# yas-sim/pyopenvino

Measured on AMD Instinct MI355X. Metric: images/sec googlenet-v1 fp32 @batch256, higher is better.
Workload: dtype f32

## Files before the change

pyopenvino_amd/csrc/pvhip_common.h:

```cpp
#pragma once
#include <hip/hip_runtime.h>
#include <cstdarg>
#include <cstdint>
#include <cstdio>

#include "../../include/pvhip.h"

namespace pvhip {

constexpr int kMaxStreams = PVHIP_MAX_STREAMS;

struct State {
    bool        ready  = false;
    int         device = -1;
    hipStream_t stream = nullptr;
    hipStream_t streams[kMaxStreams] = {};
    int         current = 0;
    bool        forked  = false;
    bool        capturing = false;
};
State& state();

struct Settings {
    int generation = 0;
    int  conv_kernel    = 0;
    bool conv_winograd  = true;
    int  conv_winograd4 = 1;
    int  conv_winograd5 = 1;
    bool conv_pointwise = true;
    bool conv_stem      = true;
    bool conv_stem_wino = false;
    int  poolconv_prio  = -1;
    int  fuse_poolconv  = 2;
    bool pool3          = true;
    int  stream_nt      = 1;
    int  stream_wg      = 16;
    int  tile_bm = 0, tile_bn = 0;
    int  wtile_m = 2, wtile_n = 1;
    int  conv_lds_pad_kb = 0;
    bool conv_nopw = false;
    int  f16_bm = 0;
    int  f16_c8_wgs = 0;
    int  f16_c8_prod = 0;
    int  f16_c8_reg = 0;
    int  f16_c8_tpw = 0;
    bool lrnpool_wave = false;
    int  dwconv_cols = 1;
    bool conv_novalid = false;
    bool conv_pw16 = false;
    int  multi_bm = 32;
    int  pw_tn = 0;
    int  pw_stagger_pct = 0;
    int  pool3_kb = 16, pool3_stage = 1, pool3_wg = 0, pool3_g = 0, pool3_s = 0, pool3_band = 0;
    bool pool3_verbose = false;
    int  pool_lds_kb = 16;
    int  wino_kb = 0;
    bool wino_small = true;
    int  wino_waves = 8;
    bool wino_ragged = true;
    bool wino_balance = true;
    int  wino_shared = 1;
    int  wino_shared_prio = 1;
    int  wino_shared_old = 1;
    bool wino_shared_odd = true;
    int  wino_shared_lag = 0;
    int  wino_shared_min_tiles = 2048;
    int  conv_ablate = 0, wino4_ablate = 0, pw_ablate = 0, stem_ablate = 0;
    int  tune[8] = {0, 0, 0, 0, 0, 0, 0, 0};
    bool pool3_tuning() const { return pool3_kb != 16 || pool3_stage != 1 || pool3_wg != 0 || pool3_g != 0; }
};
const Settings& settings();
void            load_settings();

int matmul_impl(const float* a, const float* b, float* c, int m, int n, int k, int trans_a, int trans_b, int round_f16);

int fail(int code, const char* fmt, ...);

constexpr int kWave      = 64;
constexpr int kNumCU     = 256;
constexpr int kBlock     = 256;
constexpr int kMaxBlocks = kNumCU * 8;

inline int grid_for(size_t work_items, int per_block = kBlock) {
    size_t b = (work_items + per_block - 1) / per_block;
    if (b < 1) b = 1;
    if (b > (size_t)kMaxBlocks) b = kMaxBlocks;
    return (int)b;
}

struct FastDiv {
    unsigned mul, shift, d;
};
inline FastDiv make_fastdiv(unsigned d) {
    FastDiv f{0u, 0u, d};
    if (d <= 1) return f;
    unsigned s = 0;
    while ((1ull << s) < d) ++s;
    const unsigned long long k = 31ull + s;
    f.mul   = (unsigned)(((1ull << k) + d - 1) / d);
    f.shift = s - 1;
    return f;
}
__device__ __forceinline__ unsigned fdiv(unsigned n, const FastDiv& f) {
    return f.d <= 1 ? n : (__umulhi(n, f.mul) >> f.shift);
}

__device__ __forceinline__ float max3_nan(float a, float b, float c) {
    return __builtin_elementwise_maximum(__builtin_elementwise_maximum(a, b), c);
}


struct ActBounds {
    float lo, hi;
};
__device__ __forceinline__ ActBounds act_bounds(int act, float lo, float hi) {
    ActBounds b;
    b.lo = act == 1 ? 0.0f : (act == 2 ? lo : -__builtin_inff());
    b.hi = act == 2 ? hi : __builtin_inff();
    return b;
}
__device__ __forceinline__ float act_apply(float v, const ActBounds& b) {
    v = (v < b.lo) ? b.lo : v;
    v = (v > b.hi) ? b.hi : v;
    return v;
}
template <int N>
__device__ __forceinline__ void bias_act_n(float (&v)[N], const float (&b)[N], bool has_bias, int act, const ActBounds& ab) {
    if (has_bias) {
#pragma unroll
        for (int i = 0; i < N; ++i) v[i] = v[i] + b[i];
    }
    if (act == 1) {
#pragma unroll
        for (int i = 0; i < N; ++i) v[i] = __builtin_elementwise_maximum(v[i], 0.0f);
    } else if (act != 0) {
#pragma unroll
        for (int i = 0; i < N; ++i) v[i] = (v[i] < ab.lo) ? ab.lo : v[i];
    }
    if (act == 2) {
#pragma unroll
        for (int i = 0; i < N; ++i) v[i] = (v[i] > ab.hi) ? ab.hi : v[i];
    }
}

__device__ __forceinline__ float lrn_pow_f(float d, float beta, int beta_mode) {
    if (beta_mode == 1) {
        const float s = sqrtf(d);
        return s * sqrtf(s);
    }
    if (beta_mode == 2) return sqrtf(d);
    if (beta_mode == 3) return d;
    return powf(d, beta);
}

__device__ __forceinline__ float lrn_div(float x, float d, float beta, int beta_mode) {
    if (beta_mode == 4) return x * __builtin_amdgcn_exp2f(-0.75f * __builtin_amdgcn_logf(d));
    return x / lrn_pow_f(d, beta, beta_mode);
}

inline int lrn_beta_mode(float beta, float bias) {
    if (beta == 0.75f) return bias >= 1e-20f ? 4 : 1;
    if (beta == 0.5f) return 2;
    if (beta == 1.0f) return 3;
    return 0;
}

constexpr bool kConvStoreNT = false;
constexpr bool kConvStoreSC1 = false;
typedef float pv_f4v __attribute__((ext_vector_type(4)));
typedef float pv_f2v __attribute__((ext_vector_type(2)));
__device__ __forceinline__ void conv_store1(float* p, float v) {
#if defined(__HIP_DEVICE_COMPILE__)
    if (kConvStoreSC1) { asm volatile("global_store_dword %0, %1, off sc1" :: "v"(p), "v"(v) : "memory"); return; }
#endif
    if (kConvStoreNT) __builtin_nontemporal_store(v, p);
    else *p = v;
}
__device__ __forceinline__ void conv_store2(float* p, float a, float b) {
    pv_f2v v; v.x = a; v.y = b;
#if defined(__HIP_DEVICE_COMPILE__)
    if (kConvStoreSC1) { asm volatile("global_store_dwordx2 %0, %1, off sc1" :: "v"(p), "v"(v) : "memory"); return; }
#endif
    if (kConvStoreNT) __builtin_nontemporal_store(v, reinterpret_cast<pv_f2v*>(p));
    else *reinterpret_cast<pv_f2v*>(p) = v;
}
__device__ __forceinline__ void conv_store4(float* p, float a, float b, float c, float d) {
    pv_f4v v; v.x = a; v.y = b; v.z = c; v.w = d;
#if defined(__HIP_DEVICE_COMPILE__)
    if (kConvStoreSC1) { asm volatile("global_store_dwordx4 %0, %1, off sc1" :: "v"(p), "v"(v) : "memory"); return; }
#endif
    if (kConvStoreNT) __builtin_nontemporal_store(v, reinterpret_cast<pv_f4v*>(p));
    else *reinterpret_cast<pv_f4v*>(p) = v;
}
template <class V>
__device__ __forceinline__ void conv_storev(V* p, V v) {
#if defined(__HIP_DEVICE_COMPILE__)
    if (kConvStoreSC1) {
        if constexpr (sizeof(V) == 4) { const float f_ = v[0]; asm volatile("global_store_dword %0, %1, off sc1" :: "v"(p), "v"(f_) : "memory"); }
        else if constexpr (sizeof(V) == 8) asm volatile("global_store_dwordx2 %0, %1, off sc1" :: "v"(p), "v"(v) : "memory");
        else asm volatile("global_store_dwordx4 %0, %1, off sc1" :: "v"(p), "v"(v) : "memory");
        return;
    }
#endif
    if (kConvStoreNT) __builtin_nontemporal_store(v, p);
    else *p = v;
}

typedef __attribute__((address_space(3))) void* lds_void_p;
__device__ __forceinline__ void lds_dma_b32(__amdgpu_buffer_rsrc_t r, float* dst, unsigned voff, unsigned soff) {
#if defined(__HIP_DEVICE_COMPILE__)
    const unsigned lds = (unsigned)(unsigned long)(lds_void_p)dst;
    asm volatile("s_mov_b32 m0, %0\n\ts_nop 0\n\tbuffer_load_dword %1, %2, %3 offen lds"
                 :: "s"(lds), "v"(voff), "s"(r), "s"(soff) : "memory");
#endif
}
__device__ __forceinline__ void lds_dma_b128(__amdgpu_buffer_rsrc_t r, float* dst, unsigned voff, unsigned soff) {
#if defined(__HIP_DEVICE_COMPILE__)
    const unsigned lds = (unsigned)(unsigned long)(lds_void_p)dst;
    asm volatile("s_mov_b32 m0, %0\n\ts_nop 0\n\tbuffer_load_dwordx4 %1, %2, %3 offen lds"
                 :: "s"(lds), "v"(voff), "s"(r), "s"(soff) : "memory");
#endif
}
__device__ __forceinline__ void lds_dma_wait_all() { asm volatile("s_waitcnt vmcnt(0)" ::: "memory"); }

}

#define PVHIP_REQUIRE_INIT()                                                          \
    do {                                                                              \
        if (!pvhip::state().ready)                                                    \
            return pvhip::fail(PVHIP_ENOTINIT, "%s: pvhip_init() not called", __func__); \
    } while (0)

#define PVHIP_HIP(call)                                                               \
    do {                                                                              \
        hipError_t e_ = (call);                                                       \
        if (e_ != hipSuccess)                                                         \
            return pvhip::fail(PVHIP_EHIP, "%s: %s -> %s", __func__, #call,           \
                               hipGetErrorString(e_));                                \
    } while (0)

#define PVHIP_CHECK_ARG(cond)                                                         \
    do {                                                                              \
        if (!(cond))                                                                  \
            return pvhip::fail(PVHIP_EINVAL, "%s: argument check failed: %s",         \
                               __func__, #cond);                                      \
    } while (0)

#define PVHIP_LAUNCH_CHECK()                                                          \
    do {                                                                              \
        hipError_t e_ = hipGetLastError();                                            \
        if (e_ != hipSuccess)                                                         \
            return pvhip::fail(PVHIP_EHIP, "%s: kernel launch -> %s", __func__,       \
                               hipGetErrorString(e_));                                \
    } while (0)
```

pyopenvino_amd/csrc/pvhip_norm.hip:

```cpp
#include "pvhip_common.h"

using namespace pvhip;

namespace {

constexpr bool kStreamNT = true;
template <class T>
__device__ __forceinline__ T ldnt(const T* p) { return kStreamNT ? __builtin_nontemporal_load(p) : *p; }
template <class T>
__device__ __forceinline__ void stnt(T* p, T v) { if (kStreamNT) __builtin_nontemporal_store(v, p); else *p = v; }

__device__ __forceinline__ float wave_sum(float v) {
#pragma unroll
    for (int off = kWave / 2; off > 0; off >>= 1) v += __shfl_xor(v, off, kWave);
    return v;
}

constexpr int kSoftmaxPerThread = 8;

__global__ __launch_bounds__(kBlock) void softmax_rows_kernel(const float* __restrict__ x, float* __restrict__ y,
                                                               int rows, int cols) {
    __shared__ float wave_part[kBlock / kWave];
    const int lane = threadIdx.x & (kWave - 1);
    const int wid  = threadIdx.x / kWave;
    for (int r = blockIdx.x; r < rows; r += gridDim.x) {
        const float* __restrict__ xr = x + (size_t)r * cols;
        float* __restrict__       yr = y + (size_t)r * cols;
        float e[kSoftmaxPerThread];
        float part = 0.0f;
        const bool in_regs = cols <= kBlock * kSoftmaxPerThread;
        if (in_regs) {
#pragma unroll
            for (int j = 0; j < kSoftmaxPerThread; ++j) {
                const int c = threadIdx.x + j * kBlock;
                e[j]        = (c < cols) ? expf(xr[c]) : 0.0f;
                part += e[j];
            }
        } else {
            for (int c = threadIdx.x; c < cols; c += kBlock) part += expf(xr[c]);
        }
        part = wave_sum(part);
        __syncthreads();
        if (lane == 0) wave_part[wid] = part;
        __syncthreads();
        float total = 0.0f;
#pragma unroll
        for (int wv = 0; wv < kBlock / kWave; ++wv) total += wave_part[wv];
        if (in_regs) {
#pragma unroll
            for (int j = 0; j < kSoftmaxPerThread; ++j) {
                const int c = threadIdx.x + j * kBlock;
                if (c < cols) yr[c] = e[j] / total;
            }
        } else {
            for (int c = threadIdx.x; c < cols; c += kBlock) yr[c] = expf(xr[c]) / total;
        }
    }
}

template <int SIZE, int VEC, int BETA_MODE>
__global__ __launch_bounds__(kBlock) void lrn_window_kernel(const float* __restrict__ x, float* __restrict__ y, int n,
                                                             int c, int hw, float alpha, float beta, float bias) {
    constexpr int beta_mode = BETA_MODE;
    constexpr int HALF = SIZE / 2;
    constexpr int T    = 8;
    constexpr int E    = 2 * HALF + T;
    static_assert(2 * HALF <= T, "window halo must fit in one chunk");
    typedef float vec_t __attribute__((ext_vector_type(VEC)));
    const int      cols_per_img = hw / VEC;
    const unsigned total        = (unsigned)n * (unsigned)cols_per_img;
    const unsigned stride       = gridDim.x * blockDim.x;
    const int      n_chunks     = c / T;
    const size_t   cstride      = (size_t)hw / VEC;

#define PV_LRN_OUT(j_, ch_)                                                                    \
    {                                                                                          \
        vec_t s_ = ext[(j_)] * ext[(j_)];                                                      \
        _Pragma("unroll") for (int q = 1; q < SIZE; ++q) s_ = s_ + ext[(j_) + q] * ext[(j_) + q]; \
        vec_t o_;                                                                              \
        _Pragma("unroll") for (int v = 0; v < VEC; ++v) {                                      \
            const float d_ = bias + alpha * s_[v];                                             \
            o_[v]          = lrn_div(ext[(j_) + HALF][v], d_, beta, beta_mode);                \
        }                                                                                      \
        stnt(yv + (size_t)(ch_) * cstride, o_);                                                      \
    }

    for (unsigned t = blockIdx.x * blockDim.x + threadIdx.x; t < total; t += stride) {
        const unsigned img  = t / (unsigned)cols_per_img;
        const unsigned col  = t - img * (unsigned)cols_per_img;
        const size_t   base = (size_t)img * c * hw + (size_t)col * VEC;
        const vec_t* __restrict__ xv = reinterpret_cast<const vec_t*>(x + base);
        vec_t* __restrict__       yv = reinterpret_cast<vec_t*>(y + base);
        vec_t ext[E], nxt[T];
#pragma unroll
        for (int j = 0; j < 2 * HALF; ++j) ext[j] = (vec_t)(0.0f);
#pragma unroll
        for (int j = 0; j < T; ++j) ext[2 * HALF + j] = ldnt(xv + (size_t)j * cstride);
        for (int k = 0; k + 1 < n_chunks; ++k) {
            const vec_t* __restrict__ xn = xv + (size_t)(k + 1) * T * cstride;
#pragma unroll
            for (int j = 0; j < T; ++j) nxt[j] = ldnt(xn + (size_t)j * cstride);
            if (k == 0) {
#pragma unroll
                for (int j = HALF; j < T; ++j) PV_LRN_OUT(j, j - HALF)
            } else {
                const int ch0 = k * T - HALF;
#pragma unroll
                for (int j = 0; j < T; ++j) PV_LRN_OUT(j, ch0 + j)
            }
#pragma unroll
            for (int j = 0; j < 2 * HALF; ++j) ext[j] = ext[T + j];
#pragma unroll
            for (int j = 0; j < T; ++j) ext[2 * HALF + j] = nxt[j];
        }
        {
            const int k = n_chunks - 1, ch0 = k * T - HALF;
            if (k == 0) {
#pragma unroll
                for (int j = HALF; j < T; ++j) PV_LRN_OUT(j, j - HALF)
            } else {
#pragma unroll
                for (int j = 0; j < T; ++j) PV_LRN_OUT(j, ch0 + j)
            }
#pragma unroll
            for (int j = 0; j < 2 * HALF; ++j) ext[j] = ext[T + j];
#pragma unroll
            for (int j = 0; j < T; ++j) ext[2 * HALF + j] = (vec_t)(0.0f);
#pragma unroll
            for (int j = 0; j < HALF; ++j) PV_LRN_OUT(j, c - HALF + j)
        }
    }
#undef PV_LRN_OUT
}

struct LrnPoolArgs {
    const float* x;
    float*       y;
    int   n, c, h, w, oh, ow;
    int   pt, pl, hp, wp;
    int   band_rows, n_bands;
    int   plane_l;
    float alpha, beta, bias;
    int   pool4;
    int   abl;
};

template <int SIZE, int VEC, int BETA_MODE, int ST, int NI>
__global__ __launch_bounds__(kBlock) void lrn_maxpool3x3_kernel(LrnPoolArgs a, FastDiv d_bands, FastDiv d_ow) {
    constexpr int beta_mode = BETA_MODE;
    constexpr int HALF = SIZE / 2;
    constexpr int T    = 8;
    constexpr int E    = 2 * HALF + T;
    static_assert(2 * HALF <= T, "window halo must fit in one chunk");
    typedef float vec_t __attribute__((ext_vector_type(VEC)));
    extern __shared__ __attribute__((aligned(16))) float planes[];
#ifdef PVHIP_DIAG
    const int abl = a.abl;
#else
    constexpr int abl = 0;
#endif

    const int tid = threadIdx.x;
    const int img = (int)fdiv(blockIdx.x, d_bands), band = (int)blockIdx.x - img * a.n_bands;
    const int oy0 = band * a.band_rows, oy1 = min(a.oh, oy0 + a.band_rows);
    const int rows_t = oy1 - oy0;
    const int iy_lo = max(0, oy0 * ST - a.pt), iy_hi = min(a.h, (oy1 - 1) * ST + 3 - a.pt);
    const int band_px = (iy_hi - iy_lo) * a.w;
    const int hw = a.h * a.w, ohw = a.oh * a.ow;
    const bool   active  = tid * VEC < band_px;
    const size_t cstride = (size_t)hw / VEC;
    const vec_t* __restrict__ xv =
        reinterpret_cast<const vec_t*>(a.x + (size_t)img * a.c * hw + (size_t)iy_lo * a.w + (active ? tid * VEC : 0));
    float* const mine = planes + tid * VEC;
    const int    n_chunks = a.c / T;
    const int    out_pp   = a.band_rows * a.ow;

#define PV_LRN_TO_LDS(j_, slot_)                                                               \
    {                                                                                          \
        vec_t s_ = ext[(j_)] * ext[(j_)];                                                      \
        _Pragma("unroll") for (int q = 1; q < SIZE; ++q) s_ = s_ + ext[(j_) + q] * ext[(j_) + q]; \
        vec_t o_;                                                                              \
        _Pragma("unroll") for (int v = 0; v < VEC; ++v) {                                      \
            const float d_ = a.bias + a.alpha * s_[v];                                         \
            o_[v]          = (abl & 1) ? ext[(j_) + HALF][v] : lrn_div(ext[(j_) + HALF][v], d_, a.beta, beta_mode); \
        }                                                                                      \
        if (active) *reinterpret_cast<vec_t*>(mine + (slot_) * a.plane_l) = o_;                \
    }

    unsigned tap[NI][9];
    unsigned outo[NI];
    bool     live[NI], zpad[NI];
#pragma unroll
    for (int i = 0; i < NI; ++i) {
        const unsigned rem = (unsigned)(tid + i * kBlock);
        const unsigned oyl = fdiv(rem, d_ow), ox = rem - oyl * (unsigned)a.ow;
        live[i] = (int)rem < out_pp && (int)oyl < rows_t;
        const int oy = oy0 + (int)oyl;
        const int py0 = oy * ST - a.pt, px0 = (int)ox * ST - a.pl;
        const int c0 = min(max(px0, 0), a.w - 1), c1 = min(max(px0 + 1, 0), a.w - 1), c2 = min(max(px0 + 2, 0), a.w - 1);
#pragma unroll
        for (int k = 0; k < 3; ++k) {
            const int r = (min(max(py0 + k, 0), a.h - 1) - iy_lo) * a.w;
            tap[i][3 * k + 0] = live[i] ? (unsigned)(r + c0) * 4u : 0u;
            tap[i][3 * k + 1] = live[i] ? (unsigned)(r + c1) * 4u : 0u;
            tap[i][3 * k + 2] = live[i] ? (unsigned)(r + c2) * 4u : 0u;
        }
        const bool zc = (px0 < 0) || (min((int)ox * ST + 2, a.wp - 1) - a.pl >= a.w);
        const bool zr = (py0 < 0) || (min(oy * ST + 2, a.hp - 1) - a.pt >= a.h);
        zpad[i] = zc || zr;
        outo[i] = (unsigned)(oy * a.ow) + ox;
    }
    float* const yimg = a.y + (size_t)img * a.c * ohw;
    const char* const planes_b = reinterpret_cast<const char*>(planes);
    const unsigned plane_bytes = (unsigned)a.plane_l * 4u;

    unsigned p4_row[3] = {0u, 0u, 0u}, p4_c8 = 0u, p4_out = 0u, p4_z = 0u;
    bool     p4_live = false;
    const int wv4 = tid >> 6;
    if constexpr (VEC == 4 && ST == 2) {
        if (a.pool4 != 0) {
            const int ql = tid & 63, qpr = a.ow >> 2;
            const int oyl = ql / qpr, oxq = ql - oyl * qpr;
            p4_live = oyl < rows_t;
            const int oy = oy0 + (p4_live ? oyl : 0);
            const int py0 = oy * ST, c0 = 8 * oxq;
#pragma unroll
            for (int k = 0; k < 3; ++k) p4_row[k] = (unsigned)((min(py0 + k, a.h - 1) - iy_lo) * a.w + c0) * 4u;
            p4_c8 = (unsigned)(min(c0 + 8, a.w - 1) - c0) * 4u;
            const bool zr = min(oy * ST + 2, a.hp - 1) >= a.h;
#pragma unroll
            for (int j = 0; j < 4; ++j) p4_z |= ((zr || min((4 * oxq + j) * ST + 2, a.wp - 1) >= a.w) ? 1u : 0u) << j;
            p4_out = (unsigned)(oy * a.ow + 4 * oxq);
        }
    }
    auto pool4 = [&](int n_pl, int ch0) {
        __syncthreads();
        if (p4_live && !(abl & 2)) {
            typedef float f4_t __attribute__((ext_vector_type(4)));
            for (int p = wv4; p < n_pl; p += 4) {
                const char* const pb = reinterpret_cast<const char*>(planes) + (unsigned)p * ((unsigned)a.plane_l * 4u);
                float hm[3][4];
#pragma unroll
                for (int k = 0; k < 3; ++k) {
                    const f4_t lo = *reinterpret_cast<const f4_t*>(pb + p4_row[k]), hi = *reinterpret_cast<const f4_t*>(pb + p4_row[k] + 16);
                    const float c8 = *reinterpret_cast<const float*>(pb + p4_row[k] + p4_c8);
                    hm[k][0] = max3_nan(lo[0], lo[1], lo[2]);
                    hm[k][1] = max3_nan(lo[2], lo[3], hi[0]);
                    hm[k][2] = max3_nan(hi[0], hi[1], hi[2]);
                    hm[k][3] = max3_nan(hi[2], hi[3], c8);
                }
                f4_t m;
#pragma unroll
                for (int j = 0; j < 4; ++j) {
                    const float mj = max3_nan(hm[0][j], hm[1][j], hm[2][j]);
                    m[j] = ((p4_z >> j) & 1u) ? max3_nan(mj, 0.0f, 0.0f) : mj;
                }
                if (!(abl & 4)) *reinterpret_cast<f4_t*>(a.y + (size_t)img * a.c * (a.oh * a.ow) + (size_t)(ch0 + p) * (a.oh * a.ow) + p4_out) = m;
            }
        }
        __syncthreads();
    };
    auto pool = [&](int n_pl, int ch0) {
        if constexpr (VEC == 4 && ST == 2) {
            if (a.pool4 != 0) { pool4(n_pl, ch0); return; }
        }
        __syncthreads();
#pragma unroll
        for (int i = 0; i < NI; ++i) {
            if (!live[i] || (abl & 2)) continue;
            float* yo = yimg + (size_t)ch0 * ohw + outo[i];
            unsigned pb = 0u;
            for (int p = 0; p < n_pl; ++p, pb += plane_bytes, yo += ohw) {
                float h[3];
#pragma unroll
                for (int k = 0; k < 3; ++k) {
                    const float v0 = *reinterpret_cast<const float*>(planes_b + pb + tap[i][3 * k + 0]);
                    const float v1 = *reinterpret_cast<const float*>(planes_b + pb + tap[i][3 * k + 1]);
                    const float v2 = *reinterpret_cast<const float*>(planes_b + pb + tap[i][3 * k + 2]);
                    h[k] = max3_nan(v0, v1, v2);
                }
                float m = max3_nan(h[0], h[1], h[2]);
                if (zpad[i]) m = max3_nan(m, 0.0f, 0.0f);
                if (!(abl & 4)) *yo = m;
            }
        }
        __syncthreads();
    };

    vec_t ext[E], nxt[T];
#pragma unroll
    for (int j = 0; j < 2 * HALF; ++j) ext[j] = (vec_t)(0.0f);
#pragma unroll
    for (int j = 0; j < T; ++j) ext[2 * HALF + j] = ldnt(xv + (size_t)j * cstride);
    for (int k = 0; k + 1 < n_chunks; ++k) {
        const vec_t* __restrict__ xn = xv + (size_t)((abl & 8) ? 0 : (k + 1) * T) * cstride;
#pragma unroll
        for (int j = 0; j < T; ++j) nxt[j] = ldnt(xn + (size_t)j * cstride);
        if (k == 0) {
#pragma unroll
            for (int j = HALF; j < T; ++j) PV_LRN_TO_LDS(j, j - HALF)
            pool(T - HALF, 0);
        } else {
#pragma unroll
            for (int j = 0; j < T; ++j) PV_LRN_TO_LDS(j, j)
            pool(T, k * T - HALF);
        }
#pragma unroll
        for (int j = 0; j < 2 * HALF; ++j) ext[j] = ext[T + j];
#pragma unroll
        for (int j = 0; j < T; ++j) ext[2 * HALF + j] = nxt[j];
    }
    {
        const int k = n_chunks - 1;
        if (k == 0) {
#pragma unroll
            for (int j = HALF; j < T; ++j) PV_LRN_TO_LDS(j, j - HALF)
            pool(T - HALF, 0);
        } else {
#pragma unroll
            for (int j = 0; j < T; ++j) PV_LRN_TO_LDS(j, j)
            pool(T, k * T - HALF);
        }
#pragma unroll
        for (int j = 0; j < 2 * HALF; ++j) ext[j] = ext[T + j];
#pragma unroll
        for (int j = 0; j < T; ++j) ext[2 * HALF + j] = (vec_t)(0.0f);
#pragma unroll
        for (int j = 0; j < HALF; ++j) PV_LRN_TO_LDS(j, j)
        pool(HALF, a.c - HALF);
    }
#undef PV_LRN_TO_LDS
}

template <int SIZE, int VEC, int BETA_MODE, int ST, int NI>
__global__ __launch_bounds__(kBlock) void maxpool3x3_lrn_kernel(LrnPoolArgs a, FastDiv d_bands, FastDiv d_ow) {
    constexpr int beta_mode = BETA_MODE;
    constexpr int HALF = SIZE / 2;
    constexpr int T    = 8;
    typedef float vec_t __attribute__((ext_vector_type(VEC)));
    extern __shared__ __attribute__((aligned(16))) float planes[];

    const int tid = threadIdx.x;
    const int img = (int)fdiv(blockIdx.x, d_bands), band = (int)blockIdx.x - img * a.n_bands;
    const int oy0 = band * a.band_rows, oy1 = min(a.oh, oy0 + a.band_rows);
    const int rows_t = oy1 - oy0;
    const int iy_lo = max(0, oy0 * ST - a.pt), iy_hi = min(a.h, (oy1 - 1) * ST + 3 - a.pt);
    const int band_px = (iy_hi - iy_lo) * a.w;
    const int hw = a.h * a.w, ohw = a.oh * a.ow;
    const bool   active  = tid * VEC < band_px;
    const size_t cstride = (size_t)hw / VEC;
    const vec_t* __restrict__ xv =
        reinterpret_cast<const vec_t*>(a.x + (size_t)img * a.c * hw + (size_t)iy_lo * a.w + (active ? tid * VEC : 0));
    float* const mine = planes + tid * VEC;
    const int    n_chunks = a.c / T;
    const int    out_pp   = a.band_rows * a.ow;

    unsigned tap[NI][9];
    unsigned outo[NI];
    bool     live[NI], zpad[NI];
#pragma unroll
    for (int i = 0; i < NI; ++i) {
        const unsigned rem = (unsigned)(tid + i * kBlock);
        const unsigned oyl = fdiv(rem, d_ow), ox = rem - oyl * (unsigned)a.ow;
        live[i] = (int)rem < out_pp && (int)oyl < rows_t;
        const int oy = oy0 + (int)oyl;
        const int py0 = oy * ST - a.pt, px0 = (int)ox * ST - a.pl;
        const int c0 = min(max(px0, 0), a.w - 1), c1 = min(max(px0 + 1, 0), a.w - 1), c2 = min(max(px0 + 2, 0), a.w - 1);
#pragma unroll
        for (int k = 0; k < 3; ++k) {
            const int r = (min(max(py0 + k, 0), a.h - 1) - iy_lo) * a.w;
            tap[i][3 * k + 0] = live[i] ? (unsigned)(r + c0) * 4u : 0u;
            tap[i][3 * k + 1] = live[i] ? (unsigned)(r + c1) * 4u : 0u;
            tap[i][3 * k + 2] = live[i] ? (unsigned)(r + c2) * 4u : 0u;
        }
        const bool zc = (px0 < 0) || (min((int)ox * ST + 2, a.wp - 1) - a.pl >= a.w);
        const bool zr = (py0 < 0) || (min(oy * ST + 2, a.hp - 1) - a.pt >= a.h);
        zpad[i] = zc || zr;
        outo[i] = (unsigned)(oy * a.ow) + ox;
    }
    float* const yimg = a.y + (size_t)img * a.c * ohw;
    const char* const planes_b = reinterpret_cast<const char*>(planes);
    const unsigned plane_bytes = (unsigned)a.plane_l * 4u;

    float win[NI][SIZE];
#pragma unroll
    for (int i = 0; i < NI; ++i)
#pragma unroll
        for (int q = 0; q < SIZE; ++q) win[i][q] = 0.0f;

#define PV_PUSH_EMIT(i_, v_, ch_)                                                              \
    {                                                                                          \
        _Pragma("unroll") for (int q = 0; q + 1 < SIZE; ++q) win[i_][q] = win[i_][q + 1];      \
        win[i_][SIZE - 1] = (v_);                                                              \
        if ((ch_) >= HALF) {                                                                   \
            float s_ = win[i_][0] * win[i_][0];                                                \
            _Pragma("unroll") for (int q = 1; q < SIZE; ++q) s_ = s_ + win[i_][q] * win[i_][q]; \
            const float d_ = a.bias + a.alpha * s_;                                            \
            yimg[(size_t)((ch_) - HALF) * ohw + outo[i_]] = lrn_div(win[i_][HALF], d_, a.beta, beta_mode);    \
        }                                                                                      \
    }

    vec_t cur[T], nxt[T];
#pragma unroll
    for (int j = 0; j < T; ++j) cur[j] = ldnt(xv + (size_t)j * cstride);
    for (int k = 0; k < n_chunks; ++k) {
        if (k + 1 < n_chunks) {
            const vec_t* __restrict__ xn = xv + (size_t)(k + 1) * T * cstride;
#pragma unroll
            for (int j = 0; j < T; ++j) nxt[j] = ldnt(xn + (size_t)j * cstride);
        }
        if (active) {
#pragma unroll
            for (int j = 0; j < T; ++j) *reinterpret_cast<vec_t*>(mine + j * a.plane_l) = cur[j];
        }
        __syncthreads();
#pragma unroll
        for (int i = 0; i < NI; ++i) {
            if (!live[i]) continue;
            unsigned pb = 0u;
#pragma unroll
            for (int p = 0; p < T; ++p, pb += plane_bytes) {
                float h[3];
#pragma unroll
                for (int q = 0; q < 3; ++q) {
                    const float v0 = *reinterpret_cast<const float*>(planes_b + pb + tap[i][3 * q + 0]);
                    const float v1 = *reinterpret_cast<const float*>(planes_b + pb + tap[i][3 * q + 1]);
                    const float v2 = *reinterpret_cast<const float*>(planes_b + pb + tap[i][3 * q + 2]);
                    h[q] = max3_nan(v0, v1, v2);
                }
                float m = max3_nan(h[0], h[1], h[2]);
                if (zpad[i]) m = max3_nan(m, 0.0f, 0.0f);
                const float pooled = m;
                PV_PUSH_EMIT(i, pooled, k * T + p)
            }
        }
        __syncthreads();
#pragma unroll
        for (int j = 0; j < T; ++j) cur[j] = nxt[j];
    }
#pragma unroll
    for (int i = 0; i < NI; ++i) {
        if (!live[i]) continue;
#pragma unroll
        for (int j = 0; j < HALF; ++j) PV_PUSH_EMIT(i, 0.0f, a.c + j)
    }
#undef PV_PUSH_EMIT
}

typedef float floatx32 __attribute__((ext_vector_type(32)));

struct PoolLrnConvArgs {
    LrnPoolArgs  p;
    const float* cw;
    const float* cbias;
    float*       y;
    int   k_out, act;
    float act_lo, act_hi;
};

template <int BETA_MODE, int ST, int KT>
__global__ __launch_bounds__(kBlock) void maxpool3x3_lrn_conv1x1_kernel(PoolLrnConvArgs ca, FastDiv d_bands, FastDiv d_ow) {
    constexpr int beta_mode = BETA_MODE;
    constexpr int SIZE = 5, HALF = SIZE / 2, T = 8, VEC = 4;
    typedef float vec_t __attribute__((ext_vector_type(VEC)));
    extern __shared__ __attribute__((aligned(16))) float planes[];
    const LrnPoolArgs& a = ca.p;
    float* const wl = planes + T * a.plane_l;

    const int tid = threadIdx.x;
    const int lane = tid & (kWave - 1);
    const int img = (int)fdiv(blockIdx.x, d_bands), band = (int)blockIdx.x - img * a.n_bands;
    const int oy0 = band * a.band_rows, oy1 = min(a.oh, oy0 + a.band_rows);
    const int rows_t = oy1 - oy0;
    const int iy_lo = max(0, oy0 * ST - a.pt), iy_hi = min(a.h, (oy1 - 1) * ST + 3 - a.pt);
    const int band_px = (iy_hi - iy_lo) * a.w;
    const int hw = a.h * a.w, ohw = a.oh * a.ow;
    const bool   active  = tid * VEC < band_px;
    const size_t cstride = (size_t)hw / VEC;
    const vec_t* __restrict__ xv =
        reinterpret_cast<const vec_t*>(a.x + (size_t)img * a.c * hw + (size_t)iy_lo * a.w + (active ? tid * VEC : 0));
    float* const mine = planes + tid * VEC;
    const int    n_chunks = a.c / T;
    const int    out_pp   = a.band_rows * a.ow;

    for (int e = tid; e < a.c * 32 * KT; e += kBlock) {
        const int c = e / (32 * KT), k = e - c * (32 * KT);
        wl[e] = k < ca.k_out ? ca.cw[(size_t)k * a.c + c] : 0.0f;
    }

    unsigned tap[9];
    unsigned outo;
    bool     live, zpad;
    {
        const unsigned rem = (unsigned)tid;
        const unsigned oyl = fdiv(rem, d_ow), ox = rem - oyl * (unsigned)a.ow;
        live = (int)rem < out_pp && (int)oyl < rows_t;
        const int oy = oy0 + (int)oyl;
        const int py0 = oy * ST - a.pt, px0 = (int)ox * ST - a.pl;
        const int c0 = min(max(px0, 0), a.w - 1), c1 = min(max(px0 + 1, 0), a.w - 1), c2 = min(max(px0 + 2, 0), a.w - 1);
#pragma unroll
        for (int k = 0; k < 3; ++k) {
            const int r = (min(max(py0 + k, 0), a.h - 1) - iy_lo) * a.w;
            tap[3 * k + 0] = live ? (unsigned)(r + c0) * 4u : 0u;
            tap[3 * k + 1] = live ? (unsigned)(r + c1) * 4u : 0u;
            tap[3 * k + 2] = live ? (unsigned)(r + c2) * 4u : 0u;
        }
        const bool zc = (px0 < 0) || (min((int)ox * ST + 2, a.wp - 1) - a.pl >= a.w);
        const bool zr = (py0 < 0) || (min(oy * ST + 2, a.hp - 1) - a.pt >= a.h);
        zpad = zc || zr;
        outo = live ? (unsigned)(oy * a.ow) + ox : 0xffffffffu;
    }
    const char* const planes_b = reinterpret_cast<const char*>(planes);
    const unsigned plane_bytes = (unsigned)a.plane_l * 4u;
    const float* const wl_lane = wl + (lane & 31);

    float win[SIZE];
#pragma unroll
    for (int q = 0; q < SIZE; ++q) win[q] = 0.0f;
    floatx32 acc[KT];
#pragma unroll
    for (int kt = 0; kt < KT; ++kt)
#pragma unroll
        for (int r = 0; r < 32; ++r) acc[kt][r] = 0.0f;

#define PV_PUSH_MFMA(v_, ch_)                                                                  \
    {                                                                                          \
        _Pragma("unroll") for (int q = 0; q + 1 < SIZE; ++q) win[q] = win[q + 1];              \
        win[SIZE - 1] = (v_);                                                                  \
        if ((ch_) >= HALF) {                                                                   \
            float s_ = win[0] * win[0];                                                        \
            _Pragma("unroll") for (int q = 1; q < SIZE; ++q) s_ = s_ + win[q] * win[q];        \
            const float d_ = a.bias + a.alpha * s_;                                            \
            const float o_ = live ? lrn_div(win[HALF], d_, a.beta, beta_mode) : 0.0f;          \
            const float* const wc_ = wl_lane + ((ch_) - HALF) * (32 * KT);                     \
            _Pragma("unroll") for (int kt = 0; kt < KT; ++kt)                                  \
                acc[kt] = __builtin_amdgcn_mfma_f32_32x32x1f32(wc_[32 * kt], o_, acc[kt], 0, 0, 0); \
        }                                                                                      \
    }

    vec_t cur[T], nxt[T];
#pragma unroll
    for (int j = 0; j < T; ++j) cur[j] = ldnt(xv + (size_t)j * cstride);
    for (int k = 0; k < n_chunks; ++k) {
        if (k + 1 < n_chunks) {
            const vec_t* __restrict__ xn = xv + (size_t)(k + 1) * T * cstride;
#pragma unroll
            for (int j = 0; j < T; ++j) nxt[j] = ldnt(xn + (size_t)j * cstride);
        }
        if (active) {
#pragma unroll
            for (int j = 0; j < T; ++j) *reinterpret_cast<vec_t*>(mine + j * a.plane_l) = cur[j];
        }
        __syncthreads();
        {
            unsigned pb = 0u;
#pragma unroll
            for (int p = 0; p < T; ++p, pb += plane_bytes) {
                float h[3];
#pragma unroll
                for (int q = 0; q < 3; ++q) {
                    const float v0 = *reinterpret_cast<const float*>(planes_b + pb + tap[3 * q + 0]);
                    const float v1 = *reinterpret_cast<const float*>(planes_b + pb + tap[3 * q + 1]);
                    const float v2 = *reinterpret_cast<const float*>(planes_b + pb + tap[3 * q + 2]);
                    h[q] = max3_nan(v0, v1, v2);
                }
                float m = max3_nan(h[0], h[1], h[2]);
                if (zpad) m = max3_nan(m, 0.0f, 0.0f);
                PV_PUSH_MFMA(m, k * T + p)
            }
        }
        __syncthreads();
#pragma unroll
        for (int j = 0; j < T; ++j) cur[j] = nxt[j];
    }
#pragma unroll
    for (int j = 0; j < HALF; ++j) PV_PUSH_MFMA(0.0f, a.c + j)
#undef PV_PUSH_MFMA

    const int h2 = lane >> 5;
    unsigned outo_b[2];
    outo_b[0] = (unsigned)__shfl((int)outo, lane & 31, kWave);
    outo_b[1] = (unsigned)__shfl((int)outo, 32 + (lane & 31), kWave);
    float* const yimg = ca.y + (size_t)img * ca.k_out * ohw;
    const ActBounds ab = act_bounds(ca.act, ca.act_lo, ca.act_hi);
#pragma unroll
    for (int kt = 0; kt < KT; ++kt) {
        float bv[16];
#pragma unroll
        for (int v = 0; v < 16; ++v) {
            const int kk = 32 * kt + 8 * (v >> 2) + 4 * h2 + (v & 3);
            bv[v] = (ca.cbias != nullptr && kk < ca.k_out) ? ca.cbias[kk] : 0.0f;
        }
#pragma unroll
        for (int b = 0; b < 2; ++b) {
            float vv[16];
#pragma unroll
            for (int v = 0; v < 16; ++v) vv[v] = acc[kt][16 * b + v];
            bias_act_n<16>(vv, bv, ca.cbias != nullptr, ca.act, ab);
            if (outo_b[b] != 0xffffffffu) {
#pragma unroll
                for (int v = 0; v < 16; ++v) {
                    const int kk = 32 * kt + 8 * (v >> 2) + 4 * h2 + (v & 3);
                    if (kk < ca.k_out) yimg[(size_t)kk * ohw + outo_b[b]] = vv[v];
                }
            }
        }
    }
}

struct LrnPoolWaveArgs {
    const float* x;
    float*       y;
    int   n, c, h, w, oh, ow;
    int   R, n_bands, rows_in;
    int   cg, n_groups;
    int   lpr, op;
    long  n_items;
    float alpha, beta, bias;
};

template <int BETA_MODE>
__global__ __launch_bounds__(kBlock) void lrn_maxpool3x3_wave_kernel(LrnPoolWaveArgs a) {
    constexpr int T = 4;
    typedef float vec4 __attribute__((ext_vector_type(4)));
    struct V8 { vec4 lo, hi; };
    extern __shared__ __attribute__((aligned(16))) float wave_planes[];
    const int lane = threadIdx.x & (kWave - 1);
    const int wid  = __builtin_amdgcn_readfirstlane(threadIdx.x / kWave);
    const long item = (long)blockIdx.x * (kBlock / kWave) + wid;
    if (item >= a.n_items) return;
    const int g    = (int)(item % a.n_groups);
    const long ib  = item / a.n_groups;
    const int band = (int)(ib % a.n_bands), img = (int)(ib / a.n_bands);
    const int oy0  = band * a.R;
    const int iy0  = 2 * oy0;
    const int c0   = g * a.cg;
    const int hw = a.h * a.w, ohw = a.oh * a.ow;
    const int plane_l = a.rows_in * a.w;
    float* const lds = wave_planes + (size_t)wid * T * plane_l;

    const int  lrow = lane / a.lpr, lcol = (lane - lrow * a.lpr) * 8;
    const bool lact = lrow < a.rows_in && iy0 + lrow < a.h;
    const float* const xl = a.x + (size_t)img * a.c * hw + (size_t)(lact ? (iy0 + lrow) * a.w + lcol : 0);
    float* const lmine = lds + lrow * a.w + lcol;
    const bool lwrite = lrow < a.rows_in;

    const int  prow = lane / a.op, pj = lane - prow * a.op;
    const int  oy = oy0 + prow, ox = 2 * pj;
    const bool pact = prow < a.R && oy < a.oh && ox < a.ow;
    const bool second = ox + 1 < a.ow;
    unsigned roff[3];
#pragma unroll
    for (int k = 0; k < 3; ++k) {
        const int r = 2 * prow + k;
        roff[k] = (unsigned)(((pact && iy0 + r < a.h) ? r : 2 * (pact ? prow : 0)) * a.w + 4 * (pact ? pj : 0));
    }
    const bool col4 = 4 * pj + 4 < a.w;
    float* const yout = a.y + ((size_t)img * a.c) * ohw + (size_t)(pact ? oy * a.ow + ox : 0);

    auto load8 = [&](int ch) -> V8 {
        V8 v;
        if (lact && ch >= 0 && ch < a.c) {
            const vec4* p = reinterpret_cast<const vec4*>(xl + (size_t)ch * hw);
            v.lo = ldnt(p); v.hi = ldnt(p + 1);
        } else {
            v.lo = (vec4)(0.0f); v.hi = (vec4)(0.0f);
        }
        return v;
    };
    V8 win[5], nxt[T];
#pragma unroll
    for (int q = 0; q < 5; ++q) { win[q].lo = (vec4)(0.0f); win[q].hi = (vec4)(0.0f); }
    const int n_chunks = a.cg / T + 1;
#pragma unroll
    for (int j = 0; j < T; ++j) nxt[j] = load8(c0 - 2 + j);
    for (int i = 0; i < n_chunks; ++i) {
        V8 cur[T];
#pragma unroll
        for (int j = 0; j < T; ++j) cur[j] = nxt[j];
        if (i + 1 < n_chunks) {
#pragma unroll
            for (int j = 0; j < T; ++j) nxt[j] = load8(c0 - 2 + T * (i + 1) + j);
        }
#pragma unroll
        for (int j = 0; j < T; ++j) {
#pragma unroll
            for (int q = 0; q < 4; ++q) win[q] = win[q + 1];
            win[4] = cur[j];
            if (i >= 1) {
                vec4 slo = win[0].lo * win[0].lo, shi = win[0].hi * win[0].hi;
#pragma unroll
                for (int q = 1; q < 5; ++q) { slo = slo + win[q].lo * win[q].lo; shi = shi + win[q].hi * win[q].hi; }
                vec4 olo, ohi;
#pragma unroll
                for (int v = 0; v < 4; ++v) {
                    olo[v] = lrn_div(win[2].lo[v], a.bias + a.alpha * slo[v], a.beta, BETA_MODE);
                    ohi[v] = lrn_div(win[2].hi[v], a.bias + a.alpha * shi[v], a.beta, BETA_MODE);
                }
                if (lwrite) {
                    *reinterpret_cast<vec4*>(lmine + j * plane_l) = olo;
                    *reinterpret_cast<vec4*>(lmine + j * plane_l + 4) = ohi;
                }
            }
        }
        if (i == 0) continue;
        __builtin_amdgcn_wave_barrier();
        const int ch0 = c0 + T * (i - 1);
        if (pact) {
#pragma unroll
            for (int p = 0; p < T; ++p) {
                const float* const pl = lds + p * plane_l;
                float m0[3], m1[3];
#pragma unroll
                for (int k = 0; k < 3; ++k) {
                    const vec4  v  = *reinterpret_cast<const vec4*>(pl + roff[k]);
                    const float v4 = col4 ? pl[roff[k] + 4] : v[3];
                    m0[k] = max3_nan(v[0], v[1], v[2]);
                    m1[k] = max3_nan(v[2], v[3], v4);
                }
                const float r0 = max3_nan(m0[0], m0[1], m0[2]), r1 = max3_nan(m1[0], m1[1], m1[2]);
                float* const yo = yout + (size_t)(ch0 + p) * ohw;
                if (second && (a.ow & 1) == 0) *reinterpret_cast<float2*>(yo) = make_float2(r0, r1);
                else { yo[0] = r0; if (second) yo[1] = r1; }
            }
        }
        __builtin_amdgcn_wave_barrier();
    }
}

bool plan_lrn_pool_wave(int n, int c, int h, int w, int size, float beta, float bias, int oh, int ow, int kh, int kw, int sh, int sw, int pt, int pl,
                        int pb, int pr, LrnPoolWaveArgs& a, int& bm) {
    if (n <= 0 || c < 8 || c % 4 != 0 || h < 3 || w < 8 || w % 8 != 0 || oh <= 0 || ow <= 0) return false;
    if (size != 5 || kh != 3 || kw != 3 || sh != 2 || sw != 2 || pt != 0 || pl != 0 || pb != 0 || pr != 0) return false;
    if (2 * (oh - 1) > h - 1 || 2 * (ow - 1) > w - 1 || 2 * (ow - 1) + 2 > w) return false;
    if ((unsigned long long)n * c * h * w >= (1ull << 31)) return false;
    bm = lrn_beta_mode(beta, bias);
    if (bm != 4 && bm != 1) return false;
    const int lpr = w / 8;
    const int R = (kWave / lpr - 1) / 2;
    const int op = (ow + 1) / 2;
    if (R < 1 || R * op > kWave) return false;
    int cg = 0;
    for (int cand = 64; cand >= 16; cand -= 4)
        if (c % cand == 0) { cg = cand; break; }
    if (cg == 0) return false;
    a.n = n; a.c = c; a.h = h; a.w = w; a.oh = oh; a.ow = ow;
    a.R = R; a.n_bands = (oh + R - 1) / R; a.rows_in = 2 * R + 1;
    a.cg = cg; a.n_groups = c / cg; a.lpr = lpr; a.op = op;
    a.n_items = (long)n * a.n_bands * a.n_groups;
    return (size_t)4 * 4 * a.rows_in * w * sizeof(float) <= 64 * 1024;
}

bool plan_lrn_pool(int n, int c, int h, int w, int size, float beta, float bias, int oh, int ow, int kh, int kw, int sh, int sw,
                   int pt, int pl, int pb, int pr, LrnPoolArgs& a, int& vec, int& bm, size_t& lds) {
    if (n <= 0 || c < 8 || c % 8 != 0 || h <= 0 || w <= 0 || oh <= 0 || ow <= 0) return false;
    if (size != 5 || kh != 3 || kw != 3 || sh != sw || (sh != 1 && sh != 2)) return false;
    if (pt < 0 || pl < 0 || pb < 0 || pr < 0 || pt > 2 || pl > 2) return false;
    if ((oh - 1) * sh > pt + h - 1 || (ow - 1) * sw > pl + w - 1) return false;
    if ((unsigned long long)n * c * h * w >= (1ull << 31)) return false;
    bm = lrn_beta_mode(beta, bias);
    if (bm != 4 && bm != 1) return false;
    vec = (w % 4 == 0) ? 4 : 1;
    int rows = (kBlock * vec / w - 3) / sh + 1;
    if (kBlock * vec / w < 3 && h >= 3) return false;
    if (rows < 1) return false;
    if (rows > oh) rows = oh;
    int bands = (oh + rows - 1) / rows;
    rows  = (oh + bands - 1) / bands;
    bands = (oh + rows - 1) / rows;
    int in_rows = (rows - 1) * sh + 3;
    if (in_rows > h) in_rows = h;
    if (in_rows * w > kBlock * vec) return false;
    a.n = n; a.c = c; a.h = h; a.w = w; a.oh = oh; a.ow = ow; a.pt = pt; a.pl = pl; a.hp = h + pt + pb; a.wp = w + pl + pr;
    a.band_rows = rows; a.n_bands = bands;
    if ((rows * ow + kBlock - 1) / kBlock > 4) return false;
    a.plane_l   = (in_rows * w + 3) & ~3;
    lds         = (size_t)8 * a.plane_l * sizeof(float);
    return lds <= 64 * 1024 && (long long)n * bands < (1ll << 31);
}

__global__ __launch_bounds__(kBlock) void lrn_generic_kernel(const float* __restrict__ x, float* __restrict__ y, int n,
                                                              int c, int hw, int size, float alpha, float beta,
                                                              float bias, int beta_mode) {
    const size_t total  = (size_t)n * c * hw;
    const size_t stride = (size_t)gridDim.x * blockDim.x;
    const int    half   = size / 2;
    for (size_t e = (size_t)blockIdx.x * blockDim.x + threadIdx.x; e < total; e += stride) {
        const size_t p   = e % hw;
        const size_t q   = e / hw;
        const int    ch  = (int)(q % c);
        const size_t img = q / c;
        int lo = ch - half, hi = ch + half + 1;
        if (lo < 0) lo = 0;
        if (hi > c) hi = c;
        float s = 0.0f;
        for (int k = lo; k < hi; ++k) {
            const float v = x[(img * c + k) * hw + p];
            s             = (k == lo) ? v * v : s + v * v;
        }
        const float d = bias + alpha * s;
        y[e]          = lrn_div(x[e], d, beta, beta_mode);
    }
}

template <int SIZE, int BETA_MODE>
void launch_lrn_window_b(const float* x, float* y, int n, int c, int hw, float alpha, float beta, float bias) {
    if (hw % 4 == 0) {
        const size_t cols = (size_t)n * (hw / 4);
        hipLaunchKernelGGL((lrn_window_kernel<SIZE, 4, BETA_MODE>), dim3(grid_for(cols)), dim3(kBlock), 0, state().stream, x, y,
                           n, c, hw, alpha, beta, bias);
    } else {
        const size_t cols = (size_t)n * hw;
        hipLaunchKernelGGL((lrn_window_kernel<SIZE, 1, BETA_MODE>), dim3(grid_for(cols)), dim3(kBlock), 0, state().stream, x, y,
                           n, c, hw, alpha, beta, bias);
    }
}

template <int SIZE>
void launch_lrn_window(const float* x, float* y, int n, int c, int hw, float alpha, float beta, float bias, int bm) {
    switch (bm) {
        case 1: launch_lrn_window_b<SIZE, 1>(x, y, n, c, hw, alpha, beta, bias); break;
        case 2: launch_lrn_window_b<SIZE, 2>(x, y, n, c, hw, alpha, beta, bias); break;
        case 3: launch_lrn_window_b<SIZE, 3>(x, y, n, c, hw, alpha, beta, bias); break;
        case 4: launch_lrn_window_b<SIZE, 4>(x, y, n, c, hw, alpha, beta, bias); break;
        default: launch_lrn_window_b<SIZE, 0>(x, y, n, c, hw, alpha, beta, bias); break;
    }
}

}

extern "C" {

int pvhip_softmax_rows_f32(const float* x, float* y, int rows, int cols) {
    PVHIP_REQUIRE_INIT();
    PVHIP_CHECK_ARG(rows >= 0 && cols >= 0);
    if (rows == 0 || cols == 0) return PVHIP_OK;
    PVHIP_CHECK_ARG(x != nullptr && y != nullptr);
    const int g = rows < kMaxBlocks ? rows : kMaxBlocks;
    hipLaunchKernelGGL(softmax_rows_kernel, dim3(g), dim3(kBlock), 0, state().stream, x, y, rows, cols);
    PVHIP_LAUNCH_CHECK();
    return PVHIP_OK;
}

int pvhip_lrn_f32(const float* x, float* y, int n, int c, int hw, int size, float alpha, float beta, float bias) {
    PVHIP_REQUIRE_INIT();
    PVHIP_CHECK_ARG(n >= 0 && c >= 0 && hw >= 0 && size >= 1);
    if ((size_t)n * c * hw == 0) return PVHIP_OK;
    PVHIP_CHECK_ARG(x != nullptr && y != nullptr);
    if ((unsigned long long)n * c * hw >= (1ull << 31))
        return fail(PVHIP_EUNSUPPORTED, "pvhip_lrn_f32: tensor exceeds 2^31 elements");
    const int bm = lrn_beta_mode(beta, bias);
    switch ((c % 8 == 0 && c >= 8) ? size : 0) {
        case 3: launch_lrn_window<3>(x, y, n, c, hw, alpha, beta, bias, bm); break;
        case 5: launch_lrn_window<5>(x, y, n, c, hw, alpha, beta, bias, bm); break;
        case 7: launch_lrn_window<7>(x, y, n, c, hw, alpha, beta, bias, bm); break;
        default:
            hipLaunchKernelGGL(lrn_generic_kernel, dim3(grid_for((size_t)n * c * hw)), dim3(kBlock), 0, state().stream, x, y,
                               n, c, hw, size, alpha, beta, bias, bm);
    }
    PVHIP_LAUNCH_CHECK();
    return PVHIP_OK;
}

int pvhip_lrn_maxpool_supported(int n, int c, int h, int w, int size, float beta, float bias, int oh, int ow, int kh, int kw,
                                int sh, int sw, int pad_top, int pad_left, int pad_bottom, int pad_right) {
    LrnPoolArgs a{};
    int vec = 0, bm = 0;
    size_t lds = 0;
    return plan_lrn_pool(n, c, h, w, size, beta, bias, oh, ow, kh, kw, sh, sw, pad_top, pad_left, pad_bottom, pad_right, a, vec, bm, lds) ? 1 : 0;
}

int pvhip_lrn_maxpool_f32(const float* x, float* y, int n, int c, int h, int w, int size, float alpha, float beta, float bias,
                          int oh, int ow, int kh, int kw, int sh, int sw, int pad_top, int pad_left, int pad_bottom,
                          int pad_right) {
    PVHIP_REQUIRE_INIT();
    {
        LrnPoolWaveArgs wa{};
        int wbm = 0;
        if (settings().lrnpool_wave && plan_lrn_pool_wave(n, c, h, w, size, beta, bias, oh, ow, kh, kw, sh, sw, pad_top, pad_left, pad_bottom, pad_right, wa, wbm)) {
            PVHIP_CHECK_ARG(x != nullptr && y != nullptr);
            wa.x = x; wa.y = y; wa.alpha = alpha; wa.beta = beta; wa.bias = bias;
            const long blocks = (wa.n_items + kBlock / kWave - 1) / (kBlock / kWave);
            if (blocks <= 0x7fffffffL) {
                const size_t wlds = (size_t)(kBlock / kWave) * 4 * wa.rows_in * w * sizeof(float);
                if (wbm == 4) hipLaunchKernelGGL((lrn_maxpool3x3_wave_kernel<4>), dim3((unsigned)blocks), dim3(kBlock), wlds, state().stream, wa);
                else          hipLaunchKernelGGL((lrn_maxpool3x3_wave_kernel<1>), dim3((unsigned)blocks), dim3(kBlock), wlds, state().stream, wa);
                PVHIP_LAUNCH_CHECK();
                return PVHIP_OK;
            }
        }
    }
    LrnPoolArgs a{};
    int vec = 0, bm = 0;
    size_t lds = 0;
    if (!plan_lrn_pool(n, c, h, w, size, beta, bias, oh, ow, kh, kw, sh, sw, pad_top, pad_left, pad_bottom, pad_right, a, vec, bm, lds))
        return fail(PVHIP_EUNSUPPORTED, "pvhip_lrn_maxpool_f32: shape outside the fused kernel (ask pvhip_lrn_maxpool_supported first)");
    PVHIP_CHECK_ARG(x != nullptr && y != nullptr);
    a.x = x; a.y = y; a.alpha = alpha; a.beta = beta; a.bias = bias;
    a.abl = 0;
#ifdef PVHIP_DIAG
    a.abl = settings().conv_ablate;
#endif
    a.pool4 = (vec == 4 && sh == 2 && pad_top == 0 && pad_left == 0 && ow % 4 == 0 && 2 * ow <= w && (ow / 4) * a.band_rows <= kWave && settings().tune[6] != 1) ? 1 : 0;
    const dim3 grid((unsigned)(n * a.n_bands));
    const FastDiv d_bands = make_fastdiv((unsigned)a.n_bands), d_ow = make_fastdiv((unsigned)ow);
    const int ni = (a.band_rows * ow + kBlock - 1) / kBlock;
#define PV_LP(VEC_, BM_, ST_, NI_) \
    hipLaunchKernelGGL((lrn_maxpool3x3_kernel<5, VEC_, BM_, ST_, NI_>), grid, dim3(kBlock), lds, state().stream, a, d_bands, d_ow)
#define PV_LP_NI(VEC_, BM_, ST_)                                  \
    {                                                             \
        if (ni <= 1) PV_LP(VEC_, BM_, ST_, 1);                    \
        else if (ni <= 2) PV_LP(VEC_, BM_, ST_, 2);               \
        else PV_LP(VEC_, BM_, ST_, 4);                            \
    }
    if (ni > 4) return fail(PVHIP_EUNSUPPORTED, "pvhip_lrn_maxpool_f32: more than four pooled outputs per lane and plane");
    if (vec == 4) {
        if (bm == 4) { if (sh == 1) PV_LP_NI(4, 4, 1) else PV_LP_NI(4, 4, 2) }
        else         { if (sh == 1) PV_LP_NI(4, 1, 1) else PV_LP_NI(4, 1, 2) }
    } else {
        if (bm == 4) { if (sh == 1) PV_LP_NI(1, 4, 1) else PV_LP_NI(1, 4, 2) }
        else         { if (sh == 1) PV_LP_NI(1, 1, 1) else PV_LP_NI(1, 1, 2) }
    }
#undef PV_LP_NI
#undef PV_LP
    PVHIP_LAUNCH_CHECK();
    return PVHIP_OK;
}

int pvhip_maxpool_lrn_supported(int n, int c, int h, int w, int oh, int ow, int kh, int kw, int sh, int sw, int pad_top, int pad_left,
                                int pad_bottom, int pad_right, int size, float beta, float bias) {
    LrnPoolArgs a{};
    int vec = 0, bm = 0;
    size_t lds = 0;
    return plan_lrn_pool(n, c, h, w, size, beta, bias, oh, ow, kh, kw, sh, sw, pad_top, pad_left, pad_bottom, pad_right, a, vec, bm, lds) ? 1 : 0;
}

int pvhip_maxpool_lrn_f32(const float* x, float* y, int n, int c, int h, int w, int oh, int ow, int kh, int kw, int sh, int sw,
                          int pad_top, int pad_left, int pad_bottom, int pad_right, int size, float alpha, float beta, float bias) {
    PVHIP_REQUIRE_INIT();
    LrnPoolArgs a{};
    int vec = 0, bm = 0;
    size_t lds = 0;
    if (!plan_lrn_pool(n, c, h, w, size, beta, bias, oh, ow, kh, kw, sh, sw, pad_top, pad_left, pad_bottom, pad_right, a, vec, bm, lds))
        return fail(PVHIP_EUNSUPPORTED, "pvhip_maxpool_lrn_f32: shape outside the fused kernel (ask pvhip_maxpool_lrn_supported first)");
    PVHIP_CHECK_ARG(x != nullptr && y != nullptr);
    a.x = x; a.y = y; a.alpha = alpha; a.beta = beta; a.bias = bias;
    const dim3 grid((unsigned)(n * a.n_bands));
    const FastDiv d_bands = make_fastdiv((unsigned)a.n_bands), d_ow = make_fastdiv((unsigned)ow);
    const int ni = (a.band_rows * ow + kBlock - 1) / kBlock;
    if (ni > 4) return fail(PVHIP_EUNSUPPORTED, "pvhip_maxpool_lrn_f32: more than four pooled outputs per lane and plane");
#define PV_PL(VEC_, BM_, ST_, NI_) \
    hipLaunchKernelGGL((maxpool3x3_lrn_kernel<5, VEC_, BM_, ST_, NI_>), grid, dim3(kBlock), lds, state().stream, a, d_bands, d_ow)
#define PV_PL_NI(VEC_, BM_, ST_)                                  \
    {                                                             \
        if (ni <= 1) PV_PL(VEC_, BM_, ST_, 1);                    \
        else if (ni <= 2) PV_PL(VEC_, BM_, ST_, 2);               \
        else PV_PL(VEC_, BM_, ST_, 4);                            \
    }
    if (vec == 4) {
        if (bm == 4) { if (sh == 1) PV_PL_NI(4, 4, 1) else PV_PL_NI(4, 4, 2) }
        else         { if (sh == 1) PV_PL_NI(4, 1, 1) else PV_PL_NI(4, 1, 2) }
    } else {
        if (bm == 4) { if (sh == 1) PV_PL_NI(1, 4, 1) else PV_PL_NI(1, 4, 2) }
        else         { if (sh == 1) PV_PL_NI(1, 1, 1) else PV_PL_NI(1, 1, 2) }
    }
#undef PV_PL_NI
#undef PV_PL
    PVHIP_LAUNCH_CHECK();
    return PVHIP_OK;
}

static bool plan_pool_lrn_conv(int n, int c, int h, int w, int oh, int ow, int kh, int kw, int sh, int sw, int pt, int pl, int pb, int pr, int size,
                               float beta, float bias, int k_out, LrnPoolArgs& a, int& bm, size_t& lds) {
    int vec = 0;
    if (!plan_lrn_pool(n, c, h, w, size, beta, bias, oh, ow, kh, kw, sh, sw, pt, pl, pb, pr, a, vec, bm, lds)) return false;
    if (vec != 4 || a.band_rows * ow > kBlock || k_out <= 0 || k_out > 64 || c > 64) return false;
    if ((unsigned long long)n * k_out * oh * ow >= (1ull << 31)) return false;
    lds += (size_t)c * 32 * ((k_out + 31) / 32) * sizeof(float);
    return lds <= 64 * 1024;
}

int pvhip_maxpool_lrn_conv1x1_supported(int n, int c, int h, int w, int oh, int ow, int kh, int kw, int sh, int sw, int pad_top, int pad_left,
                                        int pad_bottom, int pad_right, int size, float beta, float bias, int k_out) {
    LrnPoolArgs a{};
    int bm = 0;
    size_t lds = 0;
    return plan_pool_lrn_conv(n, c, h, w, oh, ow, kh, kw, sh, sw, pad_top, pad_left, pad_bottom, pad_right, size, beta, bias, k_out, a, bm, lds) ? 1 : 0;
}

int pvhip_maxpool_lrn_conv1x1_f32(const float* x, const float* w_oihw, float* y, int n, int c, int h, int w, int oh, int ow, int kh, int kw, int sh, int sw,
                                  int pad_top, int pad_left, int pad_bottom, int pad_right, int size, float alpha, float beta, float bias,
                                  int k_out, const float* conv_bias, int act, float act_lo, float act_hi) {
    PVHIP_REQUIRE_INIT();
    PoolLrnConvArgs ca{};
    int bm = 0;
    size_t lds = 0;
    if (!plan_pool_lrn_conv(n, c, h, w, oh, ow, kh, kw, sh, sw, pad_top, pad_left, pad_bottom, pad_right, size, beta, bias, k_out, ca.p, bm, lds))
        return fail(PVHIP_EUNSUPPORTED, "pvhip_maxpool_lrn_conv1x1_f32: shape outside the fused kernel (ask pvhip_maxpool_lrn_conv1x1_supported first)");
    PVHIP_CHECK_ARG(x != nullptr && w_oihw != nullptr && y != nullptr && act >= 0 && act <= 2);
    ca.p.x = x; ca.p.y = nullptr; ca.p.alpha = alpha; ca.p.beta = beta; ca.p.bias = bias;
    ca.cw = w_oihw; ca.cbias = conv_bias; ca.y = y; ca.k_out = k_out; ca.act = act; ca.act_lo = act_lo; ca.act_hi = act_hi;
    const dim3 grid((unsigned)(n * ca.p.n_bands));
    const FastDiv d_bands = make_fastdiv((unsigned)ca.p.n_bands), d_ow = make_fastdiv((unsigned)ow);
    const int kt = (k_out + 31) / 32;
#define PV_PLC(BM_, ST_, KT_) hipLaunchKernelGGL((maxpool3x3_lrn_conv1x1_kernel<BM_, ST_, KT_>), grid, dim3(kBlock), lds, state().stream, ca, d_bands, d_ow)
    if (bm == 4) {
        if (sh == 1) { if (kt == 1) PV_PLC(4, 1, 1); else PV_PLC(4, 1, 2); }
        else         { if (kt == 1) PV_PLC(4, 2, 1); else PV_PLC(4, 2, 2); }
    } else {
        if (sh == 1) { if (kt == 1) PV_PLC(1, 1, 1); else PV_PLC(1, 1, 2); }
        else         { if (kt == 1) PV_PLC(1, 2, 1); else PV_PLC(1, 2, 2); }
    }
#undef PV_PLC
    PVHIP_LAUNCH_CHECK();
    return PVHIP_OK;
}


}
```

pyopenvino_amd/csrc/pvhip_runtime.hip:

```cpp
#include <cstdlib>
#include <cstring>
#include <map>
#include <mutex>
#include <unordered_map>
#include <vector>

#include "pvhip_common.h"

namespace pvhip {

State& state() {
    static State s;
    return s;
}

static Settings g_settings;
const Settings& settings() {
    if (g_settings.generation == 0) load_settings();
    return g_settings;
}

void load_settings() {
    Settings s;
    s.generation = g_settings.generation + 1;
    auto env   = [](const char* name) -> const char* { const char* e = getenv(name); return (e != nullptr && e[0] != 0) ? e : nullptr; };
    auto is0   = [&](const char* name) { const char* e = env(name); return e != nullptr && e[0] == '0'; };
    auto num   = [&](const char* name, int dflt) { const char* e = env(name); return e != nullptr ? atoi(e) : dflt; };
    auto tri   = [&](const char* name) { const char* e = env(name); return e == nullptr ? 1 : (e[0] == '0' ? 0 : (e[0] == 'f' ? 2 : 1)); };
    s.conv_winograd  = !is0("PVHIP_CONV_WINOGRAD");
    s.conv_winograd4 = tri("PVHIP_CONV_WINOGRAD4");
    s.conv_winograd5 = tri("PVHIP_CONV_WINOGRAD5");
    s.conv_pointwise = !is0("PVHIP_CONV_POINTWISE");
    s.conv_stem      = !is0("PVHIP_CONV_STEM");
    { const char* e = env("PVHIP_CONV_STEM_WINO"); s.conv_stem_wino = e != nullptr && e[0] == '1'; }
    for (int i = 0; i < 8; ++i) {
        char name[16];
        snprintf(name, sizeof(name), "PVHIP_TUNE%d", i);
        s.tune[i] = num(name, 0);
    }
    if (const char* e = env("PVHIP_FUSE_POOLCONV")) s.fuse_poolconv = e[0] == '0' ? 0 : (e[0] == '4' ? 4 : (e[0] == '1' ? 1 : 2));
    s.pool3 = !(env("PVHIP_POOL3") != nullptr && num("PVHIP_POOL3", 1) == 0);
    s.stream_nt = num("PVHIP_STREAM_NT", 1);
    s.stream_wg = num("PVHIP_STREAM_WG", 16);
    if (s.stream_wg < 1) s.stream_wg = 1;
    if (s.stream_wg > 64) s.stream_wg = 64;
    s.conv_lds_pad_kb = num("PVHIP_CONV_LDS_PAD_KB", 0);
    s.conv_nopw = env("PVHIP_CONV_NOPW") != nullptr;
    s.conv_novalid = env("PVHIP_CONV_NOVALID") != nullptr;
    s.dwconv_cols = (int)num("PVHIP_DWCONV_COLS", 1);
    { const int b = num("PVHIP_CONV_F16_BM", 0); s.f16_bm = (b == 32 || b == 64 || b == 128) ? b : 0; }
    s.f16_c8_wgs = num("PVHIP_CONV_F16_C8_WGS", 0);
    s.f16_c8_prod = num("PVHIP_CONV_F16_C8_PROD", 0);
    s.f16_c8_reg = num("PVHIP_CONV_F16_C8_REG", 0);
    s.f16_c8_tpw = num("PVHIP_CONV_F16_C8_TPW", 0);
    s.lrnpool_wave = num("PVHIP_LRNPOOL_WAVE", 0) != 0;
    { const int v = num("PVHIP_CONV_MULTI_BM", 32); s.multi_bm = (v == 64 || v == 128) ? v : 32; }
    s.pw_stagger_pct = num("PVHIP_PW_STAGGER", 0);
    s.pw_tn = num("PVHIP_PW_TN", 0);
    s.pool3_kb    = num("PVHIP_POOL3_KB", 16);
    s.pool3_stage = num("PVHIP_POOL3_STAGE", 1) != 0;
    s.pool3_wg    = num("PVHIP_POOL3_WG", 0);
    if (const char* e = env("PVHIP_POOL3_CFG")) {
        int g = 0, sg = 0, band = 0;
        if (sscanf(e, "%d,%d,%d", &g, &sg, &band) == 3 && g > 0 && sg > 0 && band > 0) { s.pool3_g = g; s.pool3_s = sg; s.pool3_band = band; }
    }
    s.pool3_verbose = env("PVHIP_POOL3_VERBOSE") != nullptr;
    s.pool_lds_kb   = num("PVHIP_POOL_LDS_KB", 16);
    { const int v = num("PVHIP_WINO_KB", 0); s.wino_kb = (v == 32 || v == 64) ? v : 0; }
    s.wino_small = !is0("PVHIP_WINO_SMALL");
    s.wino_waves = num("PVHIP_WINO_WAVES", 8) == 4 ? 4 : 8;
    s.wino_balance = num("PVHIP_WINO_BALANCE", 1) != 0;
    s.wino_ragged = num("PVHIP_WINO_RAGGED", 1) != 0;
    s.wino_shared = num("PVHIP_WINO_SHARED", 1);
    s.wino_shared_min_tiles = num("PVHIP_WINO_SHARED_MIN_TILES", 2048);
    s.wino_shared_lag = num("PVHIP_WINO_SHARED_LAG", 0);
    s.wino_shared_prio = num("PVHIP_WINO_SHARED_PRIO", 1);
    s.wino_shared_odd = num("PVHIP_WINO_SHARED_ODD", 1) != 0;
    s.poolconv_prio = num("PVHIP_POOLCONV_PRIO", -1);
    s.wino_shared_old = num("PVHIP_WINO_SHARED_OLD", 1);
#ifdef PVHIP_DIAG
    if (const char* e = env("PVHIP_CONV_KERNEL")) s.conv_kernel = strcmp(e, "lds") == 0 ? 1 : (strcmp(e, "wave") == 0 ? 2 : 0);
    if (const char* e = env("PVHIP_CONV_TILE")) {
        int bm = 0, bn = 0;
        if (sscanf(e, "%dx%d", &bm, &bn) == 2 && (bm == 32 || bm == 64 || bm == 128) && (bn == 128 || bn == 256)) { s.tile_bm = bm; s.tile_bn = bn; }
    }
    if (const char* e = env("PVHIP_CONV_WTILE")) sscanf(e, "%dx%d", &s.wtile_m, &s.wtile_n);
    s.conv_pw16 = env("PVHIP_CONV_PW") != nullptr;
    s.conv_ablate  = num("PVHIP_CONV_ABLATE", 0);
    s.wino4_ablate = num("PVHIP_WINO4_ABLATE", 0);
    s.pw_ablate    = num("PVHIP_PW_ABLATE", 0);
    s.stem_ablate  = num("PVHIP_STEM_ABLATE", 0);
#endif
    g_settings = s;
}

static thread_local char g_err[512] = "no error";

int fail(int code, const char* fmt, ...) {
    va_list ap;
    va_start(ap, fmt);
    vsnprintf(g_err, sizeof(g_err), fmt, ap);
    va_end(ap);
    return code;
}

namespace {
struct Pool {
    std::mutex                                  mu;
    struct Live { size_t bytes; int epoch; bool captured; };
    std::unordered_map<void*, Live>             live;
    std::map<size_t, std::vector<void*>>        cached;
    std::vector<std::pair<void*, size_t>>       deferred;
    int                                                     next_epoch = 1, current_epoch = 0;
    std::unordered_map<int, std::vector<std::pair<void*, size_t>>> parked;
    size_t                                      bytes_live = 0, bytes_cached = 0;
    std::vector<std::pair<void*, size_t>>       capture_keep;
};
Pool& pool() {
    static Pool p;
    return p;
}
inline size_t round_up(size_t b) {
    const size_t q = 512;
    return b == 0 ? q : (b + q - 1) / q * q;
}

int sync_all_streams() {
    State& s = state();
    for (int i = 0; i < kMaxStreams; ++i)
        if (s.streams[i] != nullptr) {
            hipError_t e = hipStreamSynchronize(s.streams[i]);
            if (e != hipSuccess) return fail(PVHIP_EHIP, "hipStreamSynchronize(stream %d) -> %s", i, hipGetErrorString(e));
        }
    Pool& p = pool();
    std::lock_guard<std::mutex> g(p.mu);
    for (auto& blk : p.deferred) {
        p.cached[blk.second].push_back(blk.first);
        p.bytes_cached += blk.second;
    }
    p.deferred.clear();
    s.forked = s.current != 0;
    return PVHIP_OK;
}

struct HostBlocks {
    std::mutex               mu;
    std::map<uintptr_t, size_t> live;
};
HostBlocks& host_blocks() {
    static HostBlocks h;
    return h;
}
}
}

using namespace pvhip;

extern "C" {

int pvhip_abi_version(void) { return PVHIP_ABI_VERSION; }

const char* pvhip_last_error(void) { return g_err; }

int pvhip_device_count(int* count) {
    PVHIP_CHECK_ARG(count != nullptr);
    int n = 0;
    hipError_t e = hipGetDeviceCount(&n);
    if (e != hipSuccess) {
        *count = 0;
        return fail(PVHIP_EHIP, "hipGetDeviceCount -> %s", hipGetErrorString(e));
    }
    *count = n;
    return PVHIP_OK;
}

int pvhip_init(int device) {
    State& s = state();
    if (s.ready) {
        if (s.device == device) return PVHIP_OK;
        return fail(PVHIP_EINVAL, "pvhip_init: already initialised on device %d", s.device);
    }
    int n = 0;
    PVHIP_HIP(hipGetDeviceCount(&n));
    if (device < 0 || device >= n)
        return fail(PVHIP_EINVAL, "pvhip_init: device %d out of range (%d visible)", device, n);
    PVHIP_HIP(hipSetDevice(device));
    PVHIP_HIP(hipStreamCreateWithFlags(&s.streams[0], hipStreamNonBlocking));
    s.stream  = s.streams[0];
    s.current = 0;
    s.forked  = false;
    s.device = device;
    s.ready  = true;
    load_settings();
    return PVHIP_OK;
}

int pvhip_settings_reload(void) {
    load_settings();
    return PVHIP_OK;
}

int pvhip_pool_release(void) {
    PVHIP_REQUIRE_INIT();
    if (int rc = sync_all_streams()) return rc;
    Pool& p = pool();
    std::lock_guard<std::mutex> g(p.mu);
    for (auto& kv : p.cached)
        for (void* ptr : kv.second) (void)hipFree(ptr);
    p.cached.clear();
    p.bytes_cached = 0;
    return PVHIP_OK;
}

int pvhip_shutdown(void) {
    State& s = state();
    if (!s.ready) return PVHIP_OK;
    (void)pvhip_comm_destroy();
    (void)pvhip_pool_release();
    {
        HostBlocks& h = host_blocks();
        std::lock_guard<std::mutex> g(h.mu);
        for (auto& kv : h.live) (void)hipHostFree((void*)kv.first);
        h.live.clear();
    }
    {
        Pool& p = pool();
        std::lock_guard<std::mutex> g(p.mu);
        for (auto& kv : p.live) (void)hipFree(kv.first);
        p.live.clear();
        for (auto& kv : p.parked)
            for (auto& blk : kv.second) (void)hipFree(blk.first);
        p.parked.clear();
        for (auto& blk : p.deferred) (void)hipFree(blk.first);
        p.deferred.clear();
        p.current_epoch = 0;
        p.bytes_live = 0;
    }
    for (int i = 0; i < kMaxStreams; ++i)
        if (s.streams[i] != nullptr) {
            (void)hipStreamDestroy(s.streams[i]);
            s.streams[i] = nullptr;
        }
    s.stream  = nullptr;
    s.current = 0;
    s.forked  = false;
    s.ready  = false;
    s.device = -1;
    return PVHIP_OK;
}

int pvhip_device_name(char* buf, size_t buflen) {
    PVHIP_REQUIRE_INIT();
    PVHIP_CHECK_ARG(buf != nullptr && buflen > 0);
    hipDeviceProp_t prop;
    PVHIP_HIP(hipGetDeviceProperties(&prop, state().device));
    const char* name = prop.name[0] != 0 ? prop.name : (strncmp(prop.gcnArchName, "gfx950", 6) == 0 ? "AMD Instinct MI355X-class (gfx950)" : "AMD GPU");
    snprintf(buf, buflen, "%s (%s, %d CUs)", name, prop.gcnArchName, prop.multiProcessorCount);
    return PVHIP_OK;
}

int pvhip_malloc(void** ptr, size_t bytes) {
    PVHIP_REQUIRE_INIT();
    PVHIP_CHECK_ARG(ptr != nullptr);
    const size_t rb = round_up(bytes);
    Pool&        p  = pool();
    std::lock_guard<std::mutex> g(p.mu);
    auto it = p.cached.find(rb);
    if (it != p.cached.end() && !it->second.empty()) {
        *ptr = it->second.back();
        it->second.pop_back();
        p.bytes_cached -= rb;
    } else {
        if (state().capturing)
            return fail(PVHIP_EHIP, "pvhip_malloc(%zu bytes): the pool has no such block while a pass is being captured into a graph "
                                    "(run the pass eagerly first: steady-state inference allocates nothing new)", rb);
        void*      d = nullptr;
        hipError_t e = hipMalloc(&d, rb);
        if (e != hipSuccess) {
            (void)hipGetLastError();
            for (int i = 0; i < kMaxStreams; ++i)
                if (state().streams[i] != nullptr) (void)hipStreamSynchronize(state().streams[i]);
            for (auto& blk : p.deferred) {
                p.cached[blk.second].push_back(blk.first);
                p.bytes_cached += blk.second;
            }
            p.deferred.clear();
            for (auto& kv : p.cached)
                for (void* c : kv.second) (void)hipFree(c);
            p.cached.clear();
            p.bytes_cached = 0;
            e = hipMalloc(&d, rb);
            if (e != hipSuccess)
                return fail(PVHIP_EHIP, "pvhip_malloc(%zu bytes) -> %s", rb, hipGetErrorString(e));
        }
        *ptr = d;
    }
    p.live[*ptr] = Pool::Live{rb, p.current_epoch, state().capturing};
    p.bytes_live += rb;
    return PVHIP_OK;
}

int pvhip_free(void* ptr) {
    if (ptr == nullptr) return PVHIP_OK;
    if (!state().ready) return PVHIP_OK;
    Pool& p = pool();
    std::lock_guard<std::mutex> g(p.mu);
    auto it = p.live.find(ptr);
    if (it == p.live.end()) return fail(PVHIP_EINVAL, "pvhip_free: %p is not a live pvhip block", ptr);
    const size_t rb    = it->second.bytes;
    const int    epoch = it->second.epoch;
    const bool   captured = it->second.captured;
    p.live.erase(it);
    p.bytes_live -= rb;
    if (state().capturing && captured) {
        p.capture_keep.emplace_back(ptr, rb);
        return PVHIP_OK;
    }
    if (epoch != 0) {
        auto open = p.parked.find(epoch);
        if (open != p.parked.end()) {
            open->second.emplace_back(ptr, rb);
            return PVHIP_OK;
        }
    } else if (state().forked) {
        p.deferred.emplace_back(ptr, rb);
        return PVHIP_OK;
    }
    p.cached[rb].push_back(ptr);
    p.bytes_cached += rb;
    return PVHIP_OK;
}

int pvhip_pool_epoch_begin(int* epoch) {
    PVHIP_REQUIRE_INIT();
    PVHIP_CHECK_ARG(epoch != nullptr);
    Pool& p = pool();
    std::lock_guard<std::mutex> g(p.mu);
    *epoch          = p.next_epoch++;
    p.current_epoch = *epoch;
    p.parked[*epoch];
    return PVHIP_OK;
}

int pvhip_pool_epoch_dispatched(void) {
    PVHIP_REQUIRE_INIT();
    Pool& p = pool();
    std::lock_guard<std::mutex> g(p.mu);
    p.current_epoch = 0;
    return PVHIP_OK;
}

int pvhip_pool_epoch_end(int epoch) {
    PVHIP_REQUIRE_INIT();
    Pool& p = pool();
    std::lock_guard<std::mutex> g(p.mu);
    auto it = p.parked.find(epoch);
    if (it == p.parked.end()) return fail(PVHIP_EINVAL, "pvhip_pool_epoch_end: epoch %d is not open", epoch);
    for (auto& blk : it->second) {
        p.cached[blk.second].push_back(blk.first);
        p.bytes_cached += blk.second;
    }
    p.parked.erase(it);
    if (p.current_epoch == epoch) p.current_epoch = 0;
    return PVHIP_OK;
}

int pvhip_pool_stats(size_t* bytes_in_use, size_t* bytes_cached) {
    Pool& p = pool();
    std::lock_guard<std::mutex> g(p.mu);
    if (bytes_in_use) *bytes_in_use = p.bytes_live;
    if (bytes_cached) *bytes_cached = p.bytes_cached;
    return PVHIP_OK;
}

int pvhip_memcpy_h2d(void* dst, const void* src, size_t bytes) {
    PVHIP_REQUIRE_INIT();
    if (bytes == 0) return PVHIP_OK;
    PVHIP_CHECK_ARG(dst != nullptr && src != nullptr);
    PVHIP_HIP(hipMemcpyAsync(dst, src, bytes, hipMemcpyHostToDevice, state().stream));
    PVHIP_HIP(hipStreamSynchronize(state().stream));
    return PVHIP_OK;
}

int pvhip_memcpy_d2h(void* dst, const void* src, size_t bytes) {
    PVHIP_REQUIRE_INIT();
    if (bytes == 0) return PVHIP_OK;
    PVHIP_CHECK_ARG(dst != nullptr && src != nullptr);
    PVHIP_HIP(hipMemcpyAsync(dst, src, bytes, hipMemcpyDeviceToHost, state().stream));
    PVHIP_HIP(hipStreamSynchronize(state().stream));
    if (state().forked && state().current == 0) return sync_all_streams();
    return PVHIP_OK;
}

void* pvhip_host_alloc(size_t bytes) {
    if (!state().ready || bytes == 0) return nullptr;
    void* p = nullptr;
    if (hipHostMalloc(&p, bytes, hipHostMallocDefault) != hipSuccess) { (void)hipGetLastError(); return nullptr; }
    HostBlocks& h = host_blocks();
    std::lock_guard<std::mutex> g(h.mu);
    h.live[(uintptr_t)p] = bytes;
    return p;
}

int pvhip_host_free(void* p) {
    PVHIP_REQUIRE_INIT();
    if (p == nullptr) return PVHIP_OK;
    {
        HostBlocks& h = host_blocks();
        std::lock_guard<std::mutex> g(h.mu);
        if (h.live.erase((uintptr_t)p) == 0) return fail(PVHIP_EINVAL, "pvhip_host_free: %p is not a live pvhip_host_alloc block", p);
    }
    PVHIP_HIP(hipHostFree(p));
    return PVHIP_OK;
}

int pvhip_host_stats(size_t* blocks, size_t* bytes) {
    HostBlocks& h = host_blocks();
    std::lock_guard<std::mutex> g(h.mu);
    size_t total = 0;
    for (auto& kv : h.live) total += kv.second;
    if (blocks) *blocks = h.live.size();
    if (bytes) *bytes = total;
    return PVHIP_OK;
}

int pvhip_memcpy_h2d_async(void* dst, const void* src, size_t bytes) {
    PVHIP_REQUIRE_INIT();
    if (bytes == 0) return PVHIP_OK;
    PVHIP_CHECK_ARG(dst != nullptr && src != nullptr);
    if (state().capturing) return fail(PVHIP_EINVAL, "pvhip_memcpy_h2d_async: a pass is being captured into a graph (uploads stay outside it)");
    {
        HostBlocks& h = host_blocks();
        std::lock_guard<std::mutex> g(h.mu);
        const uintptr_t a = (uintptr_t)src;
        auto it = h.live.upper_bound(a);
        const bool inside = it != h.live.begin() && (--it, a + bytes <= it->first + it->second);
        if (!inside)
            return fail(PVHIP_EINVAL, "pvhip_memcpy_h2d_async: source %p (+%zu bytes) is not page-locked memory from pvhip_host_alloc", src, bytes);
    }
    PVHIP_HIP(hipMemcpyAsync(dst, src, bytes, hipMemcpyHostToDevice, state().stream));
    return PVHIP_OK;
}

int pvhip_memcpy_d2d(void* dst, const void* src, size_t bytes) {
    PVHIP_REQUIRE_INIT();
    if (bytes == 0) return PVHIP_OK;
    PVHIP_CHECK_ARG(dst != nullptr && src != nullptr);
    PVHIP_HIP(hipMemcpyAsync(dst, src, bytes, hipMemcpyDeviceToDevice, state().stream));
    return PVHIP_OK;
}

int pvhip_memset(void* dst, int byte, size_t bytes) {
    PVHIP_REQUIRE_INIT();
    if (bytes == 0) return PVHIP_OK;
    PVHIP_CHECK_ARG(dst != nullptr);
    PVHIP_HIP(hipMemsetAsync(dst, byte, bytes, state().stream));
    return PVHIP_OK;
}

int pvhip_sync(void) {
    PVHIP_REQUIRE_INIT();
    if (state().capturing) return fail(PVHIP_EINVAL, "pvhip_sync: a pass is being captured into a graph (nothing executes until it is replayed)");
    return sync_all_streams();
}

int pvhip_stream_select(int index) {
    PVHIP_REQUIRE_INIT();
    State& s = state();
    if (index < 0 || index >= kMaxStreams)
        return fail(PVHIP_EINVAL, "pvhip_stream_select: stream %d outside 0..%d", index, kMaxStreams - 1);
    if (s.streams[index] == nullptr) PVHIP_HIP(hipStreamCreateWithFlags(&s.streams[index], hipStreamNonBlocking));
    s.stream  = s.streams[index];
    s.current = index;
    if (index != 0) s.forked = true;
    return PVHIP_OK;
}

int pvhip_stream_wait_event(void* ev) {
    PVHIP_REQUIRE_INIT();
    PVHIP_CHECK_ARG(ev != nullptr);
    PVHIP_HIP(hipStreamWaitEvent(state().stream, (hipEvent_t)ev, 0));
    return PVHIP_OK;
}

int pvhip_event_create_untimed(void** ev) {
    PVHIP_REQUIRE_INIT();
    PVHIP_CHECK_ARG(ev != nullptr);
    hipEvent_t e;
    PVHIP_HIP(hipEventCreateWithFlags(&e, hipEventDisableTiming));
    *ev = (void*)e;
    return PVHIP_OK;
}

int pvhip_event_create(void** ev) {
    PVHIP_REQUIRE_INIT();
    PVHIP_CHECK_ARG(ev != nullptr);
    hipEvent_t e;
    PVHIP_HIP(hipEventCreate(&e));
    *ev = (void*)e;
    return PVHIP_OK;
}

int pvhip_event_destroy(void* ev) {
    if (ev == nullptr || !state().ready) return PVHIP_OK;
    PVHIP_HIP(hipEventDestroy((hipEvent_t)ev));
    return PVHIP_OK;
}

int pvhip_event_record(void* ev) {
    PVHIP_REQUIRE_INIT();
    PVHIP_CHECK_ARG(ev != nullptr);
    PVHIP_HIP(hipEventRecord((hipEvent_t)ev, state().stream));
    return PVHIP_OK;
}

int pvhip_event_sync(void* ev) {
    PVHIP_REQUIRE_INIT();
    PVHIP_CHECK_ARG(ev != nullptr);
    PVHIP_HIP(hipEventSynchronize((hipEvent_t)ev));
    return PVHIP_OK;
}

int pvhip_event_elapsed_ms(void* start, void* stop, float* ms) {
    PVHIP_REQUIRE_INIT();
    PVHIP_CHECK_ARG(start != nullptr && stop != nullptr && ms != nullptr);
    PVHIP_HIP(hipEventElapsedTime(ms, (hipEvent_t)start, (hipEvent_t)stop));
    return PVHIP_OK;
}

struct GraphExec {
    hipGraphExec_t                        exec = nullptr;
    std::vector<std::pair<void*, size_t>> keep;
};

int pvhip_graph_begin_capture(void) {
    PVHIP_REQUIRE_INIT();
    if (state().capturing) return fail(PVHIP_EINVAL, "pvhip_graph_begin_capture: a capture is already open");
    PVHIP_HIP(hipStreamBeginCapture(state().stream, hipStreamCaptureModeRelaxed));
    state().capturing = true;
    return PVHIP_OK;
}

int pvhip_graph_capture_status(int* status) {
    PVHIP_REQUIRE_INIT();
    PVHIP_CHECK_ARG(status != nullptr);
    hipStreamCaptureStatus st = hipStreamCaptureStatusNone;
    PVHIP_HIP(hipStreamIsCapturing(state().stream, &st));
    *status = st == hipStreamCaptureStatusActive ? 1 : (st == hipStreamCaptureStatusInvalidated ? 2 : 0);
    return PVHIP_OK;
}

int pvhip_graph_end_capture(void** graph_exec) {
    PVHIP_REQUIRE_INIT();
    PVHIP_CHECK_ARG(graph_exec != nullptr);
    if (!state().capturing) return fail(PVHIP_EINVAL, "pvhip_graph_end_capture: no capture is open");
    state().capturing = false;
    GraphExec* ge = new GraphExec;
    {
        Pool& p = pool();
        std::lock_guard<std::mutex> g(p.mu);
        ge->keep.swap(p.capture_keep);
    }
    auto release = [&]() {
        Pool& p = pool();
        std::lock_guard<std::mutex> g(p.mu);
        for (auto& blk : ge->keep) { p.cached[blk.second].push_back(blk.first); p.bytes_cached += blk.second; }
        delete ge;
    };
    hipGraph_t g = nullptr;
    hipStreamCaptureStatus cst = hipStreamCaptureStatusNone;
    const hipError_t qe = hipStreamIsCapturing(state().stream, &cst);
    if (getenv("PVHIP_GRAPH_VERBOSE") != nullptr) fprintf(stderr, "pvhip_graph_end_capture: hipStreamIsCapturing -> %d, status %d\n", (int)qe, (int)cst);
    hipError_t e = hipStreamEndCapture(state().stream, &g);
    if (getenv("PVHIP_GRAPH_VERBOSE") != nullptr) fprintf(stderr, "pvhip_graph_end_capture: hipStreamEndCapture -> %d, graph %p\n", (int)e, (void*)g);
    if (e == hipSuccess && (g == nullptr || cst != hipStreamCaptureStatusActive)) e = hipErrorStreamCaptureInvalidated;
    if (e != hipSuccess) {
        if (g != nullptr) (void)hipGraphDestroy(g);
        release();
        (void)hipGetLastError();
        return fail(PVHIP_EHIP, "hipStreamEndCapture -> %s (capture status %d)", hipGetErrorString(e), (int)cst);
    }
    if (getenv("PVHIP_GRAPH_VERBOSE") != nullptr) {
        size_t n_nodes = 0;
        (void)hipGraphGetNodes(g, nullptr, &n_nodes);
        fprintf(stderr, "pvhip_graph_end_capture: %zu nodes\n", n_nodes);
    }
    e = hipGraphInstantiate(&ge->exec, g, nullptr, nullptr, 0);
    (void)hipGraphDestroy(g);
    if (e != hipSuccess) { release(); return fail(PVHIP_EHIP, "hipGraphInstantiate -> %s", hipGetErrorString(e)); }
    *graph_exec = (void*)ge;
    return PVHIP_OK;
}

int pvhip_graph_launch(void* graph_exec) {
    PVHIP_REQUIRE_INIT();
    PVHIP_CHECK_ARG(graph_exec != nullptr);
    PVHIP_HIP(hipGraphLaunch(static_cast<GraphExec*>(graph_exec)->exec, state().stream));
    return PVHIP_OK;
}

int pvhip_graph_destroy(void* graph_exec) {
    if (graph_exec == nullptr) return PVHIP_OK;
    GraphExec* ge = static_cast<GraphExec*>(graph_exec);
    if (state().ready) {
        (void)sync_all_streams();
        if (ge->exec != nullptr) (void)hipGraphExecDestroy(ge->exec);
        Pool& p = pool();
        std::lock_guard<std::mutex> g(p.mu);
        for (auto& blk : ge->keep) { p.cached[blk.second].push_back(blk.first); p.bytes_cached += blk.second; }
    }
    delete ge;
    return PVHIP_OK;
}

}
```

Before: 56020.

## Make LRN+maxpool kernels persistent band walkers with halo-row carry and prefetch

Turns the fused LRN+maxpool and maxpool+LRN+conv1x1 kernels into persistent workgroups, each walking a contiguous range of (image, band) items. The first channel chunk of the next band is prefetched while the current band finishes. When consecutive bands share a boundary input row, that row's LRN output is kept in extra LDS and reused, so the overlapping halo row is neither reloaded nor recomputed. The grid is sized from LDS capacity per CU, and the kernels raise their dynamic LDS limit. This adds LDS pressure, code complexity and a risk of load imbalance.

New measurement: 55080. 0.983x the previous value.

```diff
diff --git a/pyopenvino_amd/csrc/pvhip_common.h b/pyopenvino_amd/csrc/pvhip_common.h
--- a/pyopenvino_amd/csrc/pvhip_common.h
+++ b/pyopenvino_amd/csrc/pvhip_common.h
@@ -45,6 +45,7 @@
     int  f16_c8_reg = 0;
     int  f16_c8_tpw = 0;
     bool lrnpool_wave = false;
+    int  band_wgs = 0;
     int  dwconv_cols = 1;
     bool conv_novalid = false;
     bool conv_pw16 = false;
diff --git a/pyopenvino_amd/csrc/pvhip_norm.hip b/pyopenvino_amd/csrc/pvhip_norm.hip
--- a/pyopenvino_amd/csrc/pvhip_norm.hip
+++ b/pyopenvino_amd/csrc/pvhip_norm.hip
@@ -143,7 +143,34 @@
     float alpha, beta, bias;
     int   pool4;
     int   abl;
+    int   items;
+    int   carry_l;
 };
+
+struct BandGeom {
+    int img, band, oy0, oy1, iy_lo, iy_hi;
+};
+template <int ST>
+__device__ __forceinline__ BandGeom band_geom(const LrnPoolArgs& a, int item, const FastDiv& d_bands) {
+    BandGeom g;
+    g.img   = (int)fdiv((unsigned)item, d_bands);
+    g.band  = item - g.img * a.n_bands;
+    g.oy0   = g.band * a.band_rows;
+    g.oy1   = min(a.oh, g.oy0 + a.band_rows);
+    g.iy_lo = max(0, g.oy0 * ST - a.pt);
+    g.iy_hi = min(a.h, (g.oy1 - 1) * ST + 3 - a.pt);
+    return g;
+}
+template <int ST>
+__device__ __forceinline__ bool band_carried(const LrnPoolArgs& a, const BandGeom& p, const BandGeom& g) {
+    return a.carry_l != 0 && g.img == p.img && g.band == p.band + 1 && g.iy_lo == p.iy_hi - 1 && g.iy_hi - g.iy_lo >= 2 && g.oy0 * ST - a.pt >= 0;
+}
+__device__ __forceinline__ void band_range(int items, int& item, int& item_end) {
+    const int g_ = (int)gridDim.x, b_ = (int)blockIdx.x;
+    const int per = items / g_, extra = items - per * g_;
+    item     = b_ * per + min(b_, extra);
+    item_end = item + per + (b_ < extra ? 1 : 0);
+}
 
 template <int SIZE, int VEC, int BETA_MODE, int ST, int NI>
 __global__ __launch_bounds__(kBlock) void lrn_maxpool3x3_kernel(LrnPoolArgs a, FastDiv d_bands, FastDiv d_ow) {
@@ -153,12 +180,224 @@
     constexpr int E    = 2 * HALF + T;
     static_assert(2 * HALF <= T, "window halo must fit in one chunk");
     typedef float vec_t __attribute__((ext_vector_type(VEC)));
+    typedef float f4_t __attribute__((ext_vector_type(4)));
     extern __shared__ __attribute__((aligned(16))) float planes[];
 #ifdef PVHIP_DIAG
     const int abl = a.abl;
 #else
     constexpr int abl = 0;
 #endif
+
+    const int tid = threadIdx.x;
+    int item, item_end;
+    band_range(a.items, item, item_end);
+    if (item >= item_end) return;
+    const int hw = a.h * a.w, ohw = a.oh * a.ow;
+    const size_t cstride = (size_t)hw / VEC;
+    float* const mine = planes + tid * VEC;
+    float* const carry = planes + T * a.plane_l;
+    const int    n_chunks = a.c / T;
+    const int    out_pp   = a.band_rows * a.ow;
+    const char* const planes_b = reinterpret_cast<const char*>(planes);
+    const unsigned plane_bytes = (unsigned)a.plane_l * 4u;
+    const unsigned carry_b     = (unsigned)(T * a.plane_l) * 4u;
+    const int wv4 = tid >> 6;
+
+    auto src = [&](const BandGeom& g, bool carried, bool& active) -> const vec_t* {
+        active = tid * VEC < (g.iy_hi - g.iy_lo) * a.w && !(carried && tid * VEC < a.w);
+        return reinterpret_cast<const vec_t*>(a.x + (size_t)g.img * a.c * hw + (size_t)g.iy_lo * a.w + (active ? tid * VEC : (carried ? a.w : 0)));
+    };
+
+#define PV_LRN_TO_LDS(j_, slot_)                                                               \
+    {                                                                                          \
+        vec_t s_ = ext[(j_)] * ext[(j_)];                                                      \
+        _Pragma("unroll") for (int q = 1; q < SIZE; ++q) s_ = s_ + ext[(j_) + q] * ext[(j_) + q]; \
+        vec_t o_;                                                                              \
+        _Pragma("unroll") for (int v = 0; v < VEC; ++v) {                                      \
+            const float d_ = a.bias + a.alpha * s_[v];                                         \
+            o_[v]          = (abl & 1) ? ext[(j_) + HALF][v] : lrn_div(ext[(j_) + HALF][v], d_, a.beta, beta_mode); \
+        }                                                                                      \
+        if (active) *reinterpret_cast<vec_t*>(mine + (slot_) * a.plane_l) = o_;                \
+    }
+
+    BandGeom g = band_geom<ST>(a, item, d_bands);
+    bool carried = false, active;
+    const vec_t* __restrict__ xv = src(g, false, active);
+    vec_t ext[E], nxt[T];
+#pragma unroll
+    for (int j = 0; j < T; ++j) nxt[j] = ldnt(xv + (size_t)j * cstride);
+
+    for (;;) {
+        const bool     has_next = item + 1 < item_end;
+        const BandGeom gn = has_next ? band_geom<ST>(a, item + 1, d_bands) : g;
+        const bool     carry_out = has_next && band_carried<ST>(a, g, gn);
+        bool           active_n = false;
+        const vec_t* __restrict__ xvn = has_next ? src(gn, carry_out, active_n) : xv;
+
+        const int oy0 = g.oy0, iy_lo = g.iy_lo, img = g.img;
+        const int rows_t = g.oy1 - g.oy0;
+        const int last0 = (g.iy_hi - g.iy_lo - 1) * a.w;
+
+        unsigned tap[NI][9];
+        unsigned outo[NI];
+        bool     live[NI], zpad[NI];
+#pragma unroll
+        for (int i = 0; i < NI; ++i) {
+            const unsigned rem = (unsigned)(tid + i * kBlock);
+            const unsigned oyl = fdiv(rem, d_ow), ox = rem - oyl * (unsigned)a.ow;
+            live[i] = (int)rem < out_pp && (int)oyl < rows_t;
+            const int oy = oy0 + (int)oyl;
+            const int py0 = oy * ST - a.pt, px0 = (int)ox * ST - a.pl;
+            const int c0 = min(max(px0, 0), a.w - 1), c1 = min(max(px0 + 1, 0), a.w - 1), c2 = min(max(px0 + 2, 0), a.w - 1);
+#pragma unroll
+            for (int k = 0; k < 3; ++k) {
+                const int r = (min(max(py0 + k, 0), a.h - 1) - iy_lo) * a.w;
+                tap[i][3 * k + 0] = live[i] ? (unsigned)(r + c0) * 4u : 0u;
+                tap[i][3 * k + 1] = live[i] ? (unsigned)(r + c1) * 4u : 0u;
+                tap[i][3 * k + 2] = live[i] ? (unsigned)(r + c2) * 4u : 0u;
+            }
+            const bool zc = (px0 < 0) || (min((int)ox * ST + 2, a.wp - 1) - a.pl >= a.w);
+            const bool zr = (py0 < 0) || (min(oy * ST + 2, a.hp - 1) - a.pt >= a.h);
+            zpad[i] = zc || zr;
+            outo[i] = (unsigned)(oy * a.ow) + ox;
+        }
+        float* const yimg = a.y + (size_t)img * a.c * ohw;
+
+        unsigned p4_row[3] = {0u, 0u, 0u}, p4_c8 = 0u, p4_out = 0u, p4_z = 0u, p4_s0 = plane_bytes, p4_ch = 0u;
+        bool     p4_live = false;
+        if constexpr (VEC == 4 && ST == 2) {
+            if (a.pool4 != 0) {
+                const int ql = tid & 63, qpr = a.ow >> 2;
+                const int oyl = ql / qpr, oxq = ql - oyl * qpr;
+                p4_live = oyl < rows_t;
+                const int oy = oy0 + (p4_live ? oyl : 0);
+                const int py0 = oy * ST, c0 = 8 * oxq;
+#pragma unroll
+                for (int k = 0; k < 3; ++k) p4_row[k] = (unsigned)((min(py0 + k, a.h - 1) - iy_lo) * a.w + c0) * 4u;
+                if (carried && p4_live && oyl == 0) { p4_row[0] = carry_b + (unsigned)c0 * 4u; p4_s0 = p4_ch = (unsigned)a.w * 4u; }
+                p4_c8 = (unsigned)(min(c0 + 8, a.w - 1) - c0) * 4u;
+                const bool zr = min(oy * ST + 2, a.hp - 1) >= a.h;
+#pragma unroll
+                for (int j = 0; j < 4; ++j) p4_z |= ((zr || min((4 * oxq + j) * ST + 2, a.wp - 1) >= a.w) ? 1u : 0u) << j;
+                p4_out = (unsigned)(oy * a.ow + 4 * oxq);
+            }
+        }
+        auto pool4 = [&](int n_pl, int ch0) {
+            __syncthreads();
+            for (int p = wv4; p < n_pl; p += 4) {
+                const char* const pb = planes_b + (unsigned)p * plane_bytes;
+                if (p4_live && !(abl & 2)) {
+                    float hm[3][4];
+#pragma unroll
+                    for (int k = 0; k < 3; ++k) {
+                        const char* const rb = k == 0 ? planes_b + p4_row[0] + (unsigned)p * p4_s0 + (unsigned)ch0 * p4_ch : pb + p4_row[k];
+                        const f4_t lo = *reinterpret_cast<const f4_t*>(rb), hi = *reinterpret_cast<const f4_t*>(rb + 16);
+                        const float c8 = *reinterpret_cast<const float*>(rb + p4_c8);
+                        hm[k][0] = max3_nan(lo[0], lo[1], lo[2]);
+                        hm[k][1] = max3_nan(lo[2], lo[3], hi[0]);
+                        hm[k][2] = max3_nan(hi[0], hi[1], hi[2]);
+                        hm[k][3] = max3_nan(hi[2], hi[3], c8);
+                    }
+                    f4_t m;
+#pragma unroll
+                    for (int j = 0; j < 4; ++j) {
+                        const float mj = max3_nan(hm[0][j], hm[1][j], hm[2][j]);
+                        m[j] = ((p4_z >> j) & 1u) ? max3_nan(mj, 0.0f, 0.0f) : mj;
+                    }
+                    if (!(abl & 4)) *reinterpret_cast<f4_t*>(a.y + (size_t)img * a.c * (a.oh * a.ow) + (size_t)(ch0 + p) * (a.oh * a.ow) + p4_out) = m;
+                }
+                if (carry_out) {
+                    for (int q = tid & 63; q < (a.w >> 2); q += kWave)
+                        *reinterpret_cast<f4_t*>(carry + (ch0 + p) * a.carry_l + 4 * q) = *reinterpret_cast<const f4_t*>(planes + p * a.plane_l + last0 + 4 * q);
+                }
+            }
+            __syncthreads();
+        };
+        auto pool = [&](int n_pl, int ch0) {
+            if constexpr (VEC == 4 && ST == 2) {
+                if (a.pool4 != 0) { pool4(n_pl, ch0); return; }
+            }
+            __syncthreads();
+#pragma unroll
+            for (int i = 0; i < NI; ++i) {
+                if (!live[i] || (abl & 2)) continue;
+                float* yo = yimg + (size_t)ch0 * ohw + outo[i];
+                unsigned pb = 0u;
+                for (int p = 0; p < n_pl; ++p, pb += plane_bytes, yo += ohw) {
+                    float h[3];
+#pragma unroll
+                    for (int k = 0; k < 3; ++k) {
+                        const float v0 = *reinterpret_cast<const float*>(planes_b + pb + tap[i][3 * k + 0]);
+                        const float v1 = *reinterpret_cast<const float*>(planes_b + pb + tap[i][3 * k + 1]);
+                        const float v2 = *reinterpret_cast<const float*>(planes_b + pb + tap[i][3 * k + 2]);
+                        h[k] = max3_nan(v0, v1, v2);
+                    }
+                    float m = max3_nan(h[0], h[1], h[2]);
+                    if (zpad[i]) m = max3_nan(m, 0.0f, 0.0f);
+                    if (!(abl & 4)) *yo = m;
+                }
+            }
+            __syncthreads();
+        };
+
+#pragma unroll
+        for (int j = 0; j < 2 * HALF; ++j) ext[j] = (vec_t)(0.0f);
+#pragma unroll
+        for (int j = 0; j < T; ++j) ext[2 * HALF + j] = nxt[j];
+        for (int k = 0; k + 1 < n_chunks; ++k) {
+            const vec_t* __restrict__ xn = xv + (size_t)((abl & 8) ? 0 : (k + 1) * T) * cstride;
+#pragma unroll
+            for (int j = 0; j < T; ++j) nxt[j] = ldnt(xn + (size_t)j * cstride);
+            if (k == 0) {
+#pragma unroll
+                for (int j = HALF; j < T; ++j) PV_LRN_TO_LDS(j, j - HALF)
+                pool(T - HALF, 0);
+            } else {
+#pragma unroll
+                for (int j = 0; j < T; ++j) PV_LRN_TO_LDS(j, j)
+                pool(T, k * T - HALF);
+            }
+#pragma unroll
+            for (int j = 0; j < 2 * HALF; ++j) ext[j] = ext[T + j];
+#pragma unroll
+            for (int j = 0; j < T; ++j) ext[2 * HALF + j] = nxt[j];
+        }
+        {
+            if (has_next) {
+#pragma unroll
+                for (int j = 0; j < T; ++j) nxt[j] = ldnt(xvn + (size_t)j * cstride);
+            }
+            const int k = n_chunks - 1;
+            if (k == 0) {
+#pragma unroll
+                for (int j = HALF; j < T; ++j) PV_LRN_TO_LDS(j, j - HALF)
+                pool(T - HALF, 0);
+            } else {
+#pragma unroll
+                for (int j = 0; j < T; ++j) PV_LRN_TO_LDS(j, j)
+                pool(T, k * T - HALF);
+            }
+#pragma unroll
+            for (int j = 0; j < 2 * HALF; ++j) ext[j] = ext[T + j];
+#pragma unroll
+            for (int j = 0; j < T; ++j) ext[2 * HALF + j] = (vec_t)(0.0f);
+#pragma unroll
+            for (int j = 0; j < HALF; ++j) PV_LRN_TO_LDS(j, j)
+            pool(HALF, a.c - HALF);
+        }
+        if (!has_next) break;
+        ++item; g = gn; carried = carry_out; active = active_n; xv = xvn;
+    }
+#undef PV_LRN_TO_LDS
+}
+
+template <int SIZE, int VEC, int BETA_MODE, int ST, int NI>
+__global__ __launch_bounds__(kBlock) void maxpool3x3_lrn_kernel(LrnPoolArgs a, FastDiv d_bands, FastDiv d_ow) {
+    constexpr int beta_mode = BETA_MODE;
+    constexpr int HALF = SIZE / 2;
+    constexpr int T    = 8;
+    typedef float vec_t __attribute__((ext_vector_type(VEC)));
+    extern __shared__ __attribute__((aligned(16))) float planes[];
 
     const int tid = threadIdx.x;
     const int img = (int)fdiv(blockIdx.x, d_bands), band = (int)blockIdx.x - img * a.n_bands;
@@ -175,186 +414,6 @@
     const int    n_chunks = a.c / T;
     const int    out_pp   = a.band_rows * a.ow;
 
-#define PV_LRN_TO_LDS(j_, slot_)                                                               \
-    {                                                                                          \
-        vec_t s_ = ext[(j_)] * ext[(j_)];                                                      \
-        _Pragma("unroll") for (int q = 1; q < SIZE; ++q) s_ = s_ + ext[(j_) + q] * ext[(j_) + q]; \
-        vec_t o_;                                                                              \
-        _Pragma("unroll") for (int v = 0; v < VEC; ++v) {                                      \
-            const float d_ = a.bias + a.alpha * s_[v];                                         \
-            o_[v]          = (abl & 1) ? ext[(j_) + HALF][v] : lrn_div(ext[(j_) + HALF][v], d_, a.beta, beta_mode); \
-        }                                                                                      \
-        if (active) *reinterpret_cast<vec_t*>(mine + (slot_) * a.plane_l) = o_;                \
-    }
-
-    unsigned tap[NI][9];
-    unsigned outo[NI];
-    bool     live[NI], zpad[NI];
-#pragma unroll
-    for (int i = 0; i < NI; ++i) {
-        const unsigned rem = (unsigned)(tid + i * kBlock);
-        const unsigned oyl = fdiv(rem, d_ow), ox = rem - oyl * (unsigned)a.ow;
-        live[i] = (int)rem < out_pp && (int)oyl < rows_t;
-        const int oy = oy0 + (int)oyl;
-        const int py0 = oy * ST - a.pt, px0 = (int)ox * ST - a.pl;
-        const int c0 = min(max(px0, 0), a.w - 1), c1 = min(max(px0 + 1, 0), a.w - 1), c2 = min(max(px0 + 2, 0), a.w - 1);
-#pragma unroll
-        for (int k = 0; k < 3; ++k) {
-            const int r = (min(max(py0 + k, 0), a.h - 1) - iy_lo) * a.w;
-            tap[i][3 * k + 0] = live[i] ? (unsigned)(r + c0) * 4u : 0u;
-            tap[i][3 * k + 1] = live[i] ? (unsigned)(r + c1) * 4u : 0u;
-            tap[i][3 * k + 2] = live[i] ? (unsigned)(r + c2) * 4u : 0u;
-        }
-        const bool zc = (px0 < 0) || (min((int)ox * ST + 2, a.wp - 1) - a.pl >= a.w);
-        const bool zr = (py0 < 0) || (min(oy * ST + 2, a.hp - 1) - a.pt >= a.h);
-        zpad[i] = zc || zr;
-        outo[i] = (unsigned)(oy * a.ow) + ox;
-    }
-    float* const yimg = a.y + (size_t)img * a.c * ohw;
-    const char* const planes_b = reinterpret_cast<const char*>(planes);
-    const unsigned plane_bytes = (unsigned)a.plane_l * 4u;
-
-    unsigned p4_row[3] = {0u, 0u, 0u}, p4_c8 = 0u, p4_out = 0u, p4_z = 0u;
-    bool     p4_live = false;
-    const int wv4 = tid >> 6;
-    if constexpr (VEC == 4 && ST == 2) {
-        if (a.pool4 != 0) {
-            const int ql = tid & 63, qpr = a.ow >> 2;
-            const int oyl = ql / qpr, oxq = ql - oyl * qpr;
-            p4_live = oyl < rows_t;
-            const int oy = oy0 + (p4_live ? oyl : 0);
-            const int py0 = oy * ST, c0 = 8 * oxq;
-#pragma unroll
-            for (int k = 0; k < 3; ++k) p4_row[k] = (unsigned)((min(py0 + k, a.h - 1) - iy_lo) * a.w + c0) * 4u;
-            p4_c8 = (unsigned)(min(c0 + 8, a.w - 1) - c0) * 4u;
-            const bool zr = min(oy * ST + 2, a.hp - 1) >= a.h;
-#pragma unroll
-            for (int j = 0; j < 4; ++j) p4_z |= ((zr || min((4 * oxq + j) * ST + 2, a.wp - 1) >= a.w) ? 1u : 0u) << j;
-            p4_out = (unsigned)(oy * a.ow + 4 * oxq);
-        }
-    }
-    auto pool4 = [&](int n_pl, int ch0) {
-        __syncthreads();
-        if (p4_live && !(abl & 2)) {
-            typedef float f4_t __attribute__((ext_vector_type(4)));
-            for (int p = wv4; p < n_pl; p += 4) {
-                const char* const pb = reinterpret_cast<const char*>(planes) + (unsigned)p * ((unsigned)a.plane_l * 4u);
-                float hm[3][4];
-#pragma unroll
-                for (int k = 0; k < 3; ++k) {
-                    const f4_t lo = *reinterpret_cast<const f4_t*>(pb + p4_row[k]), hi = *reinterpret_cast<const f4_t*>(pb + p4_row[k] + 16);
-                    const float c8 = *reinterpret_cast<const float*>(pb + p4_row[k] + p4_c8);
-                    hm[k][0] = max3_nan(lo[0], lo[1], lo[2]);
-                    hm[k][1] = max3_nan(lo[2], lo[3], hi[0]);
-                    hm[k][2] = max3_nan(hi[0], hi[1], hi[2]);
-                    hm[k][3] = max3_nan(hi[2], hi[3], c8);
-                }
-                f4_t m;
-#pragma unroll
-                for (int j = 0; j < 4; ++j) {
-                    const float mj = max3_nan(hm[0][j], hm[1][j], hm[2][j]);
-                    m[j] = ((p4_z >> j) & 1u) ? max3_nan(mj, 0.0f, 0.0f) : mj;
-                }
-                if (!(abl & 4)) *reinterpret_cast<f4_t*>(a.y + (size_t)img * a.c * (a.oh * a.ow) + (size_t)(ch0 + p) * (a.oh * a.ow) + p4_out) = m;
-            }
-        }
-        __syncthreads();
-    };
-    auto pool = [&](int n_pl, int ch0) {
-        if constexpr (VEC == 4 && ST == 2) {
-            if (a.pool4 != 0) { pool4(n_pl, ch0); return; }
-        }
-        __syncthreads();
-#pragma unroll
-        for (int i = 0; i < NI; ++i) {
-            if (!live[i] || (abl & 2)) continue;
-            float* yo = yimg + (size_t)ch0 * ohw + outo[i];
-            unsigned pb = 0u;
-            for (int p = 0; p < n_pl; ++p, pb += plane_bytes, yo += ohw) {
-                float h[3];
-#pragma unroll
-                for (int k = 0; k < 3; ++k) {
-                    const float v0 = *reinterpret_cast<const float*>(planes_b + pb + tap[i][3 * k + 0]);
-                    const float v1 = *reinterpret_cast<const float*>(planes_b + pb + tap[i][3 * k + 1]);
-                    const float v2 = *reinterpret_cast<const float*>(planes_b + pb + tap[i][3 * k + 2]);
-                    h[k] = max3_nan(v0, v1, v2);
-                }
-                float m = max3_nan(h[0], h[1], h[2]);
-                if (zpad[i]) m = max3_nan(m, 0.0f, 0.0f);
-                if (!(abl & 4)) *yo = m;
-            }
-        }
-        __syncthreads();
-    };
-
-    vec_t ext[E], nxt[T];
-#pragma unroll
-    for (int j = 0; j < 2 * HALF; ++j) ext[j] = (vec_t)(0.0f);
-#pragma unroll
-    for (int j = 0; j < T; ++j) ext[2 * HALF + j] = ldnt(xv + (size_t)j * cstride);
-    for (int k = 0; k + 1 < n_chunks; ++k) {
-        const vec_t* __restrict__ xn = xv + (size_t)((abl & 8) ? 0 : (k + 1) * T) * cstride;
-#pragma unroll
-        for (int j = 0; j < T; ++j) nxt[j] = ldnt(xn + (size_t)j * cstride);
-        if (k == 0) {
-#pragma unroll
-            for (int j = HALF; j < T; ++j) PV_LRN_TO_LDS(j, j - HALF)
-            pool(T - HALF, 0);
-        } else {
-#pragma unroll
-            for (int j = 0; j < T; ++j) PV_LRN_TO_LDS(j, j)
-            pool(T, k * T - HALF);
-        }
-#pragma unroll
-        for (int j = 0; j < 2 * HALF; ++j) ext[j] = ext[T + j];
-#pragma unroll
-        for (int j = 0; j < T; ++j) ext[2 * HALF + j] = nxt[j];
-    }
-    {
-        const int k = n_chunks - 1;
-        if (k == 0) {
-#pragma unroll
-            for (int j = HALF; j < T; ++j) PV_LRN_TO_LDS(j, j - HALF)
-            pool(T - HALF, 0);
-        } else {
-#pragma unroll
-            for (int j = 0; j < T; ++j) PV_LRN_TO_LDS(j, j)
-            pool(T, k * T - HALF);
-        }
-#pragma unroll
-        for (int j = 0; j < 2 * HALF; ++j) ext[j] = ext[T + j];
-#pragma unroll
-        for (int j = 0; j < T; ++j) ext[2 * HALF + j] = (vec_t)(0.0f);
-#pragma unroll
-        for (int j = 0; j < HALF; ++j) PV_LRN_TO_LDS(j, j)
-        pool(HALF, a.c - HALF);
-    }
-#undef PV_LRN_TO_LDS
-}
-
-template <int SIZE, int VEC, int BETA_MODE, int ST, int NI>
-__global__ __launch_bounds__(kBlock) void maxpool3x3_lrn_kernel(LrnPoolArgs a, FastDiv d_bands, FastDiv d_ow) {
-    constexpr int beta_mode = BETA_MODE;
-    constexpr int HALF = SIZE / 2;
-    constexpr int T    = 8;
-    typedef float vec_t __attribute__((ext_vector_type(VEC)));
-    extern __shared__ __attribute__((aligned(16))) float planes[];
-
-    const int tid = threadIdx.x;
-    const int img = (int)fdiv(blockIdx.x, d_bands), band = (int)blockIdx.x - img * a.n_bands;
-    const int oy0 = band * a.band_rows, oy1 = min(a.oh, oy0 + a.band_rows);
-    const int rows_t = oy1 - oy0;
-    const int iy_lo = max(0, oy0 * ST - a.pt), iy_hi = min(a.h, (oy1 - 1) * ST + 3 - a.pt);
-    const int band_px = (iy_hi - iy_lo) * a.w;
-    const int hw = a.h * a.w, ohw = a.oh * a.ow;
-    const bool   active  = tid * VEC < band_px;
-    const size_t cstride = (size_t)hw / VEC;
-    const vec_t* __restrict__ xv =
-        reinterpret_cast<const vec_t*>(a.x + (size_t)img * a.c * hw + (size_t)iy_lo * a.w + (active ? tid * VEC : 0));
-    float* const mine = planes + tid * VEC;
-    const int    n_chunks = a.c / T;
-    const int    out_pp   = a.band_rows * a.ow;
-
     unsigned tap[NI][9];
     unsigned outo[NI];
     bool     live[NI], zpad[NI];
@@ -459,26 +518,22 @@
 };
 
 template <int BETA_MODE, int ST, int KT>
-__global__ __launch_bounds__(kBlock) void maxpool3x3_lrn_conv1x1_kernel(PoolLrnConvArgs ca, FastDiv d_bands, FastDiv d_ow) {
+__global__ __launch_bounds__(kBlock, 2) void maxpool3x3_lrn_conv1x1_kernel(PoolLrnConvArgs ca, FastDiv d_bands, FastDiv d_ow) {
     constexpr int beta_mode = BETA_MODE;
     constexpr int SIZE = 5, HALF = SIZE / 2, T = 8, VEC = 4;
     typedef float vec_t __attribute__((ext_vector_type(VEC)));
     extern __shared__ __attribute__((aligned(16))) float planes[];
     const LrnPoolArgs& a = ca.p;
-    float* const wl = planes + T * a.plane_l;
+    float* const wl    = planes + T * a.plane_l;
+    float* const carry = wl + a.c * 32 * KT;
 
     const int tid = threadIdx.x;
     const int lane = tid & (kWave - 1);
-    const int img = (int)fdiv(blockIdx.x, d_bands), band = (int)blockIdx.x - img * a.n_bands;
-    const int oy0 = band * a.band_rows, oy1 = min(a.oh, oy0 + a.band_rows);
-    const int rows_t = oy1 - oy0;
-    const int iy_lo = max(0, oy0 * ST - a.pt), iy_hi = min(a.h, (oy1 - 1) * ST + 3 - a.pt);
-    const int band_px = (iy_hi - iy_lo) * a.w;
+    int item, item_end;
+    band_range(a.items, item, item_end);
+    if (item >= item_end) return;
     const int hw = a.h * a.w, ohw = a.oh * a.ow;
-    const bool   active  = tid * VEC < band_px;
     const size_t cstride = (size_t)hw / VEC;
-    const vec_t* __restrict__ xv =
-        reinterpret_cast<const vec_t*>(a.x + (size_t)img * a.c * hw + (size_t)iy_lo * a.w + (active ? tid * VEC : 0));
     float* const mine = planes + tid * VEC;
     const int    n_chunks = a.c / T;
     const int    out_pp   = a.band_rows * a.ow;
@@ -487,124 +542,165 @@
         const int c = e / (32 * KT), k = e - c * (32 * KT);
         wl[e] = k < ca.k_out ? ca.cw[(size_t)k * a.c + c] : 0.0f;
     }
-
-    unsigned tap[9];
-    unsigned outo;
-    bool     live, zpad;
-    {
-        const unsigned rem = (unsigned)tid;
-        const unsigned oyl = fdiv(rem, d_ow), ox = rem - oyl * (unsigned)a.ow;
-        live = (int)rem < out_pp && (int)oyl < rows_t;
-        const int oy = oy0 + (int)oyl;
-        const int py0 = oy * ST - a.pt, px0 = (int)ox * ST - a.pl;
-        const int c0 = min(max(px0, 0), a.w - 1), c1 = min(max(px0 + 1, 0), a.w - 1), c2 = min(max(px0 + 2, 0), a.w - 1);
-#pragma unroll
-        for (int k = 0; k < 3; ++k) {
-            const int r = (min(max(py0 + k, 0), a.h - 1) - iy_lo) * a.w;
-            tap[3 * k + 0] = live ? (unsigned)(r + c0) * 4u : 0u;
-            tap[3 * k + 1] = live ? (unsigned)(r + c1) * 4u : 0u;
-            tap[3 * k + 2] = live ? (unsigned)(r + c2) * 4u : 0u;
-        }
-        const bool zc = (px0 < 0) || (min((int)ox * ST + 2, a.wp - 1) - a.pl >= a.w);
-        const bool zr = (py0 < 0) || (min(oy * ST + 2, a.hp - 1) - a.pt >= a.h);
-        zpad = zc || zr;
-        outo = live ? (unsigned)(oy * a.ow) + ox : 0xffffffffu;
-    }
     const char* const planes_b = reinterpret_cast<const char*>(planes);
     const unsigned plane_bytes = (unsigned)a.plane_l * 4u;
+    const unsigned carry_b     = (unsigned)(T * a.plane_l + a.c * 32 * KT) * 4u;
     const float* const wl_lane = wl + (lane & 31);
-
-    float win[SIZE];
-#pragma unroll
-    for (int q = 0; q < SIZE; ++q) win[q] = 0.0f;
-    floatx32 acc[KT];
-#pragma unroll
-    for (int kt = 0; kt < KT; ++kt)
-#pragma unroll
-        for (int r = 0; r < 32; ++r) acc[kt][r] = 0.0f;
+    const ActBounds ab = act_bounds(ca.act, ca.act_lo, ca.act_hi);
+
+    auto src = [&](const BandGeom& g, bool carried, bool& active) -> const vec_t* {
+        active = tid * VEC < (g.iy_hi - g.iy_lo) * a.w && !(carried && tid * VEC < a.w);
+        return reinterpret_cast<const vec_t*>(a.x + (size_t)g.img * a.c * hw + (size_t)g.iy_lo * a.w + (active ? tid * VEC : (carried ? a.w : 0)));
+    };
+
+    BandGeom g = band_geom<ST>(a, item, d_bands);
+    bool carried = false, active;
+    const vec_t* __restrict__ xv = src(g, false, active);
+    vec_t cur[T], nxt[T];
+#pragma unroll
+    for (int j = 0; j < T; ++j) cur[j] = ldnt(xv + (size_t)j * cstride);
+
+    for (;;) {
+        const bool     has_next = item + 1 < item_end;
+        const BandGeom gn = has_next ? band_geom<ST>(a, item + 1, d_bands) : g;
+        const bool     carry_out = has_next && band_carried<ST>(a, g, gn);
+        bool           active_n = false;
+        const vec_t* __restrict__ xvn = has_next ? src(gn, carry_out, active_n) : xv;
+
+        const int rows_t = g.oy1 - g.oy0;
+        const int band_px = (g.iy_hi - g.iy_lo) * a.w;
+        const int last0 = band_px - a.w;
+        const bool lastrow = carry_out && tid * VEC >= last0 && tid * VEC < band_px;
+
+        unsigned tap[9], strd0 = plane_bytes, kadv0 = 0u;
+        unsigned outo;
+        bool     live, zpad;
+        {
+            const unsigned rem = (unsigned)tid;
+            const unsigned oyl = fdiv(rem, d_ow), ox = rem - oyl * (unsigned)a.ow;
+            live = (int)rem < out_pp && (int)oyl < rows_t;
+            const int oy = g.oy0 + (int)oyl;
+            const int py0 = oy * ST - a.pt, px0 = (int)ox * ST - a.pl;
+            const int c0 = min(max(px0, 0), a.w - 1), c1 = min(max(px0 + 1, 0), a.w - 1), c2 = min(max(px0 + 2, 0), a.w - 1);
+#pragma unroll
+            for (int k = 0; k < 3; ++k) {
+                const int r = (min(max(py0 + k, 0), a.h - 1) - g.iy_lo) * a.w;
+                tap[3 * k + 0] = live ? (unsigned)(r + c0) * 4u : 0u;
+                tap[3 * k + 1] = live ? (unsigned)(r + c1) * 4u : 0u;
+                tap[3 * k + 2] = live ? (unsigned)(r + c2) * 4u : 0u;
+            }
+            if (carried && live && min(max(py0, 0), a.h - 1) == g.iy_lo) {
+                tap[0] = carry_b + (unsigned)c0 * 4u; tap[1] = carry_b + (unsigned)c1 * 4u; tap[2] = carry_b + (unsigned)c2 * 4u;
+                strd0 = (unsigned)a.w * 4u; kadv0 = (unsigned)(T * a.w) * 4u;
+            }
+            const bool zc = (px0 < 0) || (min((int)ox * ST + 2, a.wp - 1) - a.pl >= a.w);
+            const bool zr = (py0 < 0) || (min(oy * ST + 2, a.hp - 1) - a.pt >= a.h);
+            zpad = zc || zr;
+            outo = live ? (unsigned)(oy * a.ow) + ox : 0xffffffffu;
+        }
+
+        float win[SIZE];
+#pragma unroll
+        for (int q = 0; q < SIZE; ++q) win[q] = 0.0f;
+        floatx32 acc[KT];
+#pragma unroll
+        for (int kt = 0; kt < KT; ++kt)
+#pragma unroll
+            for (int r = 0; r < 32; ++r) acc[kt][r] = 0.0f;
 
 #define PV_PUSH_MFMA(v_, ch_)                                                                  \
-    {                                                                                          \
-        _Pragma("unroll") for (int q = 0; q + 1 < SIZE; ++q) win[q] = win[q + 1];              \
-        win[SIZE - 1] = (v_);                                                                  \
-        if ((ch_) >= HALF) {                                                                   \
-            float s_ = win[0] * win[0];                                                        \
-            _Pragma("unroll") for (int q = 1; q < SIZE; ++q) s_ = s_ + win[q] * win[q];        \
-            const float d_ = a.bias + a.alpha * s_;                                            \
-            const float o_ = live ? lrn_div(win[HALF], d_, a.beta, beta_mode) : 0.0f;          \
-            const float* const wc_ = wl_lane + ((ch_) - HALF) * (32 * KT);                     \
-            _Pragma("unroll") for (int kt = 0; kt < KT; ++kt)                                  \
-                acc[kt] = __builtin_amdgcn_mfma_f32_32x32x1f32(wc_[32 * kt], o_, acc[kt], 0, 0, 0); \
-        }                                                                                      \
-    }
-
-    vec_t cur[T], nxt[T];
-#pragma unroll
-    for (int j = 0; j < T; ++j) cur[j] = ldnt(xv + (size_t)j * cstride);
-    for (int k = 0; k < n_chunks; ++k) {
-        if (k + 1 < n_chunks) {
-            const vec_t* __restrict__ xn = xv + (size_t)(k + 1) * T * cstride;
-#pragma unroll
-            for (int j = 0; j < T; ++j) nxt[j] = ldnt(xn + (size_t)j * cstride);
-        }
-        if (active) {
-#pragma unroll
-            for (int j = 0; j < T; ++j) *reinterpret_cast<vec_t*>(mine + j * a.plane_l) = cur[j];
-        }
-        __syncthreads();
-        {
-            unsigned pb = 0u;
-#pragma unroll
-            for (int p = 0; p < T; ++p, pb += plane_bytes) {
-                float h[3];
-#pragma unroll
-                for (int q = 0; q < 3; ++q) {
-                    const float v0 = *reinterpret_cast<const float*>(planes_b + pb + tap[3 * q + 0]);
-                    const float v1 = *reinterpret_cast<const float*>(planes_b + pb + tap[3 * q + 1]);
-                    const float v2 = *reinterpret_cast<const float*>(planes_b + pb + tap[3 * q + 2]);
-                    h[q] = max3_nan(v0, v1, v2);
+        {                                                                                      \
+            _Pragma("unroll") for (int q = 0; q + 1 < SIZE; ++q) win[q] = win[q + 1];          \
+            win[SIZE - 1] = (v_);                                                              \
+            if ((ch_) >= HALF) {                                                               \
+                float s_ = win[0] * win[0];                                                    \
+                _Pragma("unroll") for (int q = 1; q < SIZE; ++q) s_ = s_ + win[q] * win[q];    \
+                const float d_ = a.bias + a.alpha * s_;                                        \
+                const float o_ = live ? lrn_div(win[HALF], d_, a.beta, beta_mode) : 0.0f;      \
+                const float* const wc_ = wl_lane + ((ch_) - HALF) * (32 * KT);                 \
+                _Pragma("unroll") for (int kt = 0; kt < KT; ++kt)                              \
+                    acc[kt] = __builtin_amdgcn_mfma_f32_32x32x1f32(wc_[32 * kt], o_, acc[kt], 0, 0, 0); \
+            }                                                                                  \
+        }
+
+        for (int k = 0; k < n_chunks; ++k) {
+            if (k + 1 < n_chunks) {
+                const vec_t* __restrict__ xn = xv + (size_t)(k + 1) * T * cstride;
+#pragma unroll
+                for (int j = 0; j < T; ++j) nxt[j] = ldnt(xn + (size_t)j * cstride);
+            }
+            if (active) {
+#pragma unroll
+                for (int j = 0; j < T; ++j) *reinterpret_cast<vec_t*>(mine + j * a.plane_l) = cur[j];
+            }
+            __syncthreads();
+            {
+                unsigned pb = 0u, p0 = (unsigned)k * kadv0;
+#pragma unroll
+                for (int p = 0; p < T; ++p, pb += plane_bytes, p0 += strd0) {
+                    float h[3];
+#pragma unroll
+                    for (int q = 0; q < 3; ++q) {
+                        const unsigned rb = q == 0 ? p0 : pb;
+                        const float v0 = *reinterpret_cast<const float*>(planes_b + rb + tap[3 * q + 0]);
+                        const float v1 = *reinterpret_cast<const float*>(planes_b + rb + tap[3 * q + 1]);
+                        const float v2 = *reinterpret_cast<const float*>(planes_b + rb + tap[3 * q + 2]);
+                        h[q] = max3_nan(v0, v1, v2);
+                    }
+                    float m = max3_nan(h[0], h[1], h[2]);
+                    if (zpad) m = max3_nan(m, 0.0f, 0.0f);
+                    PV_PUSH_MFMA(m, k * T + p)
                 }
-                float m = max3_nan(h[0], h[1], h[2]);
-                if (zpad) m = max3_nan(m, 0.0f, 0.0f);
-                PV_PUSH_MFMA(m, k * T + p)
-            }
-        }
-        __syncthreads();
-#pragma unroll
-        for (int j = 0; j < T; ++j) cur[j] = nxt[j];
-    }
-#pragma unroll
-    for (int j = 0; j < HALF; ++j) PV_PUSH_MFMA(0.0f, a.c + j)
+            }
+            __syncthreads();
+            if (lastrow) {
+#pragma unroll
+                for (int j = 0; j < T; ++j) *reinterpret_cast<vec_t*>(carry + (k * T + j) * a.carry_l + (tid * VEC - last0)) = cur[j];
+            }
+#pragma unroll
+            for (int j = 0; j < T; ++j) cur[j] = nxt[j];
+        }
+#pragma unroll
+        for (int j = 0; j < HALF; ++j) PV_PUSH_MFMA(0.0f, a.c + j)
 #undef PV_PUSH_MFMA
 
-    const int h2 = lane >> 5;
-    unsigned outo_b[2];
-    outo_b[0] = (unsigned)__shfl((int)outo, lane & 31, kWave);
-    outo_b[1] = (unsigned)__shfl((int)outo, 32 + (lane & 31), kWave);
-    float* const yimg = ca.y + (size_t)img * ca.k_out * ohw;
-    const ActBounds ab = act_bounds(ca.act, ca.act_lo, ca.act_hi);
-#pragma unroll
-    for (int kt = 0; kt < KT; ++kt) {
-        float bv[16];
-#pragma unroll
-        for (int v = 0; v < 16; ++v) {
-            const int kk = 32 * kt + 8 * (v >> 2) + 4 * h2 + (v & 3);
-            bv[v] = (ca.cbias != nullptr && kk < ca.k_out) ? ca.cbias[kk] : 0.0f;
-        }
-#pragma unroll
-        for (int b = 0; b < 2; ++b) {
-            float vv[16];
-#pragma unroll
-            for (int v = 0; v < 16; ++v) vv[v] = acc[kt][16 * b + v];
-            bias_act_n<16>(vv, bv, ca.cbias != nullptr, ca.act, ab);
-            if (outo_b[b] != 0xffffffffu) {
-#pragma unroll
-                for (int v = 0; v < 16; ++v) {
-                    const int kk = 32 * kt + 8 * (v >> 2) + 4 * h2 + (v & 3);
-                    if (kk < ca.k_out) yimg[(size_t)kk * ohw + outo_b[b]] = vv[v];
+        if (has_next) {
+#pragma unroll
+            for (int j = 0; j < T; ++j) cur[j] = ldnt(xvn + (size_t)j * cstride);
+        }
+
+        unsigned outo_b[2];
+        outo_b[0] = (unsigned)__shfl((int)outo, lane & 31, kWave);
+        outo_b[1] = (unsigned)__shfl((int)outo, 32 + (lane & 31), kWave);
+        float* const yimg = ca.y + (size_t)g.img * ca.k_out * ohw;
+        const float* cbias = ca.cbias;
+        int          h2 = lane >> 5;
+        asm volatile("" : "+s"(cbias), "+v"(h2));
+#pragma unroll
+        for (int kt = 0; kt < KT; ++kt) {
+            float bv[16];
+#pragma unroll
+            for (int v = 0; v < 16; ++v) {
+                const int kk = 32 * kt + 8 * (v >> 2) + 4 * h2 + (v & 3);
+                bv[v] = (cbias != nullptr && kk < ca.k_out) ? cbias[kk] : 0.0f;
+            }
+#pragma unroll
+            for (int b = 0; b < 2; ++b) {
+                float vv[16];
+#pragma unroll
+                for (int v = 0; v < 16; ++v) vv[v] = acc[kt][16 * b + v];
+                bias_act_n<16>(vv, bv, cbias != nullptr, ca.act, ab);
+                if (outo_b[b] != 0xffffffffu) {
+#pragma unroll
+                    for (int v = 0; v < 16; ++v) {
+                        const int kk = 32 * kt + 8 * (v >> 2) + 4 * h2 + (v & 3);
+                        if (kk < ca.k_out) yimg[(size_t)kk * ohw + outo_b[b]] = vv[v];
+                    }
                 }
             }
         }
+        if (!has_next) break;
+        ++item; g = gn; carried = carry_out; active = active_n; xv = xvn;
     }
 }
 
@@ -726,6 +822,28 @@
         }
         __builtin_amdgcn_wave_barrier();
     }
+}
+
+constexpr size_t kLdsPerCU = 160 * 1024;
+unsigned plan_band_walk(LrnPoolArgs& a, size_t lds_base, bool can_carry, int wgs_by_regs, size_t& lds) {
+    a.items = a.n * a.n_bands;
+    const size_t carry_bytes = (size_t)a.c * a.w * sizeof(float);
+    const bool   carry = can_carry && a.n_bands > 1 && lds_base + carry_bytes <= kLdsPerCU;
+    lds = lds_base + (carry ? carry_bytes : 0);
+    int per_cu = (int)(kLdsPerCU / lds);
+    per_cu = per_cu < 1 ? 1 : (per_cu > wgs_by_regs ? wgs_by_regs : per_cu);
+    const long grid = settings().band_wgs > 0 ? settings().band_wgs : (long)kNumCU * per_cu;
+    a.carry_l = carry ? a.w : 0;
+    if (grid >= a.items) { a.carry_l = 0; lds = lds_base; return (unsigned)a.items; }
+    return (unsigned)grid;
+}
+template <auto K>
+hipError_t allow_lds(size_t lds) {
+    static size_t allowed = 64 * 1024;
+    if (lds <= allowed) return hipSuccess;
+    const hipError_t e = hipFuncSetAttribute(reinterpret_cast<const void*>(K), hipFuncAttributeMaxDynamicSharedMemorySize, (int)lds);
+    if (e == hipSuccess) allowed = lds;
+    return e;
 }
 
 bool plan_lrn_pool_wave(int n, int c, int h, int w, int size, float beta, float bias, int oh, int ow, int kh, int kw, int sh, int sw, int pt, int pl,
@@ -902,16 +1020,19 @@
     a.abl = settings().conv_ablate;
 #endif
     a.pool4 = (vec == 4 && sh == 2 && pad_top == 0 && pad_left == 0 && ow % 4 == 0 && 2 * ow <= w && (ow / 4) * a.band_rows <= kWave && settings().tune[6] != 1) ? 1 : 0;
-    const dim3 grid((unsigned)(n * a.n_bands));
+    const dim3 grid(plan_band_walk(a, lds, a.pool4 != 0, 3, lds));
     const FastDiv d_bands = make_fastdiv((unsigned)a.n_bands), d_ow = make_fastdiv((unsigned)ow);
     const int ni = (a.band_rows * ow + kBlock - 1) / kBlock;
-#define PV_LP(VEC_, BM_, ST_, NI_) \
-    hipLaunchKernelGGL((lrn_maxpool3x3_kernel<5, VEC_, BM_, ST_, NI_>), grid, dim3(kBlock), lds, state().stream, a, d_bands, d_ow)
+#define PV_LP(VEC_, BM_, ST_, NI_)                                                                                                   \
+    {                                                                                                                                \
+        PVHIP_HIP((allow_lds<lrn_maxpool3x3_kernel<5, VEC_, BM_, ST_, NI_>>(lds)));                                                    \
+        hipLaunchKernelGGL((lrn_maxpool3x3_kernel<5, VEC_, BM_, ST_, NI_>), grid, dim3(kBlock), lds, state().stream, a, d_bands, d_ow); \
+    }
 #define PV_LP_NI(VEC_, BM_, ST_)                                  \
     {                                                             \
-        if (ni <= 1) PV_LP(VEC_, BM_, ST_, 1);                    \
-        else if (ni <= 2) PV_LP(VEC_, BM_, ST_, 2);               \
-        else PV_LP(VEC_, BM_, ST_, 4);                            \
+        if (ni <= 1) PV_LP(VEC_, BM_, ST_, 1)                     \
+        else if (ni <= 2) PV_LP(VEC_, BM_, ST_, 2)                \
+        else PV_LP(VEC_, BM_, ST_, 4)                             \
     }
     if (ni > 4) return fail(PVHIP_EUNSUPPORTED, "pvhip_lrn_maxpool_f32: more than four pooled outputs per lane and plane");
     if (vec == 4) {
@@ -1000,16 +1121,20 @@
     PVHIP_CHECK_ARG(x != nullptr && w_oihw != nullptr && y != nullptr && act >= 0 && act <= 2);
     ca.p.x = x; ca.p.y = nullptr; ca.p.alpha = alpha; ca.p.beta = beta; ca.p.bias = bias;
     ca.cw = w_oihw; ca.cbias = conv_bias; ca.y = y; ca.k_out = k_out; ca.act = act; ca.act_lo = act_lo; ca.act_hi = act_hi;
-    const dim3 grid((unsigned)(n * ca.p.n_bands));
+    const dim3 grid(plan_band_walk(ca.p, lds, true, 2, lds));
     const FastDiv d_bands = make_fastdiv((unsigned)ca.p.n_bands), d_ow = make_fastdiv((unsigned)ow);
     const int kt = (k_out + 31) / 32;
-#define PV_PLC(BM_, ST_, KT_) hipLaunchKernelGGL((maxpool3x3_lrn_conv1x1_kernel<BM_, ST_, KT_>), grid, dim3(kBlock), lds, state().stream, ca, d_bands, d_ow)
+#define PV_PLC(BM_, ST_, KT_)                                                                                                     \
+    {                                                                                                                             \
+        PVHIP_HIP((allow_lds<maxpool3x3_lrn_conv1x1_kernel<BM_, ST_, KT_>>(lds)));                                                  \
+        hipLaunchKernelGGL((maxpool3x3_lrn_conv1x1_kernel<BM_, ST_, KT_>), grid, dim3(kBlock), lds, state().stream, ca, d_bands, d_ow); \
+    }
     if (bm == 4) {
-        if (sh == 1) { if (kt == 1) PV_PLC(4, 1, 1); else PV_PLC(4, 1, 2); }
-        else         { if (kt == 1) PV_PLC(4, 2, 1); else PV_PLC(4, 2, 2); }
+        if (sh == 1) { if (kt == 1) PV_PLC(4, 1, 1) else PV_PLC(4, 1, 2) }
+        else         { if (kt == 1) PV_PLC(4, 2, 1) else PV_PLC(4, 2, 2) }
     } else {
-        if (sh == 1) { if (kt == 1) PV_PLC(1, 1, 1); else PV_PLC(1, 1, 2); }
-        else         { if (kt == 1) PV_PLC(1, 2, 1); else PV_PLC(1, 2, 2); }
+        if (sh == 1) { if (kt == 1) PV_PLC(1, 1, 1) else PV_PLC(1, 1, 2) }
+        else         { if (kt == 1) PV_PLC(1, 2, 1) else PV_PLC(1, 2, 2) }
     }
 #undef PV_PLC
     PVHIP_LAUNCH_CHECK();
diff --git a/pyopenvino_amd/csrc/pvhip_runtime.hip b/pyopenvino_amd/csrc/pvhip_runtime.hip
--- a/pyopenvino_amd/csrc/pvhip_runtime.hip
+++ b/pyopenvino_amd/csrc/pvhip_runtime.hip
@@ -54,6 +54,7 @@
     s.f16_c8_reg = num("PVHIP_CONV_F16_C8_REG", 0);
     s.f16_c8_tpw = num("PVHIP_CONV_F16_C8_TPW", 0);
     s.lrnpool_wave = num("PVHIP_LRNPOOL_WAVE", 0) != 0;
+    s.band_wgs = num("PVHIP_BAND_WGS", 0);
     { const int v = num("PVHIP_CONV_MULTI_BM", 32); s.multi_bm = (v == 64 || v == 128) ? v : 32; }
     s.pw_stagger_pct = num("PVHIP_PW_STAGGER", 0);
     s.pw_tn = num("PVHIP_PW_TN", 0);
```
